# VikParuchuri/surya

Measured on AMD Instinct MI355X. Metric: text-lines/sec recognised (whole node), higher is better.
Workload: dtype bf16; 1 GPU; RecognitionPredictor device loop, 256 ragged 64x{128..512} crops/GPU, batch 256, max_tokens=48, REC-FULL synthetic weights (conditioned recipe, seed 0), tiles resident in HBM; parallelism=1 GPU, weights=conditioned

## Files before the change

### include/surya_amd.h

```cpp
#ifndef SURYA_AMD_H
#define SURYA_AMD_H
#include <stddef.h>
#include <stdint.h>

#ifdef __cplusplus
extern "C" {
#endif

#define SA_OK 0
#define SA_ERR_ARG (-1)
#define SA_ERR_SHAPE (-2)
#define SA_ERR_UNSUPPORTED (-3)
#define SA_ERR_STATE (-4)
#define SA_ERR_NOMEM (-5)

#define SA_DTYPE_F32 0
#define SA_DTYPE_BF16 1
#define SA_DTYPE_F16 2

const char* surya_amd_version(void);

typedef struct surya_rec_config {
    int32_t enc_depth, enc_hidden, enc_inter, enc_inter_pad, enc_heads;
    int32_t patch_dim, patch_dim_pad;
    int32_t merge;
    int32_t window_tokens;
    int32_t enc_out_hidden;
    uint32_t fullatt_mask;
    float enc_eps;
    int32_t vocab, dec_hidden, dec_inter, dec_layers, dec_heads, dec_kv_heads, dec_head_dim;
    float dec_eps;
    int32_t bbox_size, embed_multiplier;
    int32_t image_token_id, pad_token_id, eos_token_id;
    int32_t max_slots;
    int32_t max_kv_len;
    int32_t max_patches;
    int32_t max_prefill_tokens;
    int32_t dtype;
} surya_rec_config;

enum {
    SA_RW_PATCH = 0, SA_RW_MERGER_LN, SA_RW_FC1_W, SA_RW_FC1_B, SA_RW_FC2_W, SA_RW_FC2_B, SA_RW_IMG_H, SA_RW_IMG_W,
    SA_RW_DEC_NORM, SA_RW_TOK_EMBED, SA_RW_LM_W, SA_RW_LM_B, SA_RW_BBOX_W, SA_RW_BBOX_B, SA_RW_ENC_INVFREQ,
    SA_RW_DEC_INVFREQ, SA_RW_GLOBALS
};
enum { SA_RE_NORM1 = 0, SA_RE_QKV_W, SA_RE_QKV_B, SA_RE_PROJ_W, SA_RE_PROJ_B, SA_RE_NORM2, SA_RE_GU_W, SA_RE_GU_B,
       SA_RE_DOWN_W, SA_RE_DOWN_B, SA_RE_COUNT };
enum { SA_RD_LN1 = 0, SA_RD_QKV_W, SA_RD_QKV_B, SA_RD_O_W, SA_RD_LN2, SA_RD_GU_W, SA_RD_DOWN_W, SA_RD_COUNT };
#define SA_RW_ENC(l, k) (SA_RW_GLOBALS + (l) * SA_RE_COUNT + (k))
#define SA_RW_DEC(cfg_enc_depth, l, k) (SA_RW_GLOBALS + (cfg_enc_depth) * SA_RE_COUNT + (l) * SA_RD_COUNT + (k))
#define SA_RW_TOTAL(enc_depth, dec_layers) (SA_RW_GLOBALS + (enc_depth) * SA_RE_COUNT + (dec_layers) * SA_RD_COUNT)

typedef struct surya_rec surya_rec;

size_t surya_rec_workspace_bytes(const surya_rec_config* cfg);

int surya_rec_create(const surya_rec_config* cfg, const void* const* weights, int n_weights, surya_rec** out);
int surya_rec_destroy(surya_rec* h);

int surya_rec_plan_encoder(const surya_rec_config* cfg, const int32_t* grid_hw, int n_images, int32_t* src_row,
                           int32_t* pos_hw, int32_t* cu_window, int32_t* n_windows, int32_t* merged_src);

int surya_rec_prefill(surya_rec* h, const float* tiles, const int32_t* grid_hw, int n_images, const int32_t* input_ids,
                      const int32_t* seq_offsets, const int32_t* slot_ids, int n_seqs, void* stream);

int surya_rec_encode_ahead(surya_rec* h, const float* tiles, const int32_t* grid_hw, int n_images, void* stream);

int surya_rec_set_active(surya_rec* h, const int32_t* slots, int n_active, void* stream);

#define SA_MAX_STEPS 16
int surya_rec_decode(surya_rec* h, int n_steps, void* stream);

int surya_rec_read_outputs(surya_rec* h, int n_steps, int32_t* tokens, float* scores, int32_t* bboxes, void* stream);

int surya_rec_decode_async(surya_rec* h, int n_steps, int ring, void* stream);
int surya_rec_wait_outputs(surya_rec* h, int n_steps, int ring, int32_t* tokens, float* scores, int32_t* bboxes);

int surya_rec_preprocess(const uint8_t* pages, const void* lines, int n_lines, uint8_t* mask_arena, float* mid_arena, float* tiles,
                         int patch_size, int merge_size, float pad_value, const float* mean, const float* std, int any_poly,
                         int max_stage1_width, int pixel_stride, void* stream);

int surya_rec_encode_only(surya_rec* h, const float* tiles, const int32_t* grid_hw, int n_images, void* out, void* stream);
int surya_rec_copy_last_logits(surya_rec* h, float* dst, int max_rows, int* rows, void* stream);
int surya_rec_set_next_tokens(surya_rec* h, const int32_t* slots, const int32_t* tokens, int n, void* stream);

enum { SA_MX_QKV_W = 0, SA_MX_QKV_S, SA_MX_O_W, SA_MX_O_S, SA_MX_GU_W, SA_MX_GU_S, SA_MX_DOWN_W, SA_MX_DOWN_S, SA_MX_COUNT };
enum { SA_MX_LM_W = 0, SA_MX_LM_S, SA_MX_GLOBALS };
#define SA_MX_TOTAL(dec_layers) ((dec_layers) * SA_MX_COUNT + SA_MX_GLOBALS)
int surya_rec_set_mx_weights(surya_rec* h, const void* const* table, int n);

int surya_rec_set_kv_fp8(surya_rec* h, int on);

int surya_op_gemm(int dtype, int out_f32, int epi, const void* X, long ldx, const void* W, long ldw, void* C, long ldc,
                  const void* bias, const void* R, long ldr, int M, int N, int K, void* stream);
int surya_op_rmsnorm(int dtype, const void* x, long ldx, const void* w, void* y, long ldy, int rows, int C, float eps,
                     void* stream);
int surya_op_attn(int dtype, int head_dim, const void* q, const void* k, const void* v, void* out, const int32_t* seg_len,
                  const int64_t* q_off, const int64_t* k_off, const int64_t* v_off, const int64_t* o_off, int n_seg, int heads, int group,
                  int causal, float scale, long q_row, long q_head, long k_row, long k_head, long o_row, long o_head, void* stream);
int surya_op_decode_attn(int dtype, int head_dim, const float* qkv_part, int n_slabs, const void* qkv_bias, void* out, void* kcache,
                         void* vcache, const int32_t* active_slots, const int32_t* row_len, const float* rope_cs, int rows, int heads,
                         int kv_heads, int max_kv_len, float scale, void* stream);
int surya_op_kv8_quant_rows(int head_dim, const void* kcache, const void* vcache, const int32_t* tok_slot, const int32_t* tok_pos, int n_tokens,
                            void* k8, void* v8t, float* kscale, float* vscale, int kv_heads, int max_kv_len, void* stream);
int surya_op_decode_attn_kv8(int head_dim, const float* qkv_part, int n_slabs, const void* qkv_bias, void* out, void* k8, void* v8t,
                             float* kscale, float* vscale, const int32_t* active_slots, const int32_t* row_len, const float* rope_cs, int rows,
                             int heads, int kv_heads, int max_kv_len, float scale, void* stream);

int surya_op_gemm_splitk_bf16(const void* X, long ldx, const void* W, long ldw, float* part, int M, int N, int K, int* splitk, void* stream);
int surya_op_mx_quantize(const float* x, int rows, int K, uint8_t* q, uint8_t* scales, void* stream);
int surya_op_gemm_mx(int mode, const uint8_t* X, const uint8_t* SX, const uint8_t* W, const uint8_t* SW, int M, int N, int K,
                     float* C, int* splitk, uint8_t* q_out, uint8_t* sq_out, void* stream);

enum { SA_DET_INPUT = 0,
       SA_DET_CONV,
       SA_DET_DWCONV,
       SA_DET_GROUPED1X1,
       SA_DET_LITEMLA,
       SA_DET_UPCAT,
       SA_DET_CLASSIFY,
       SA_DET_UPSAMPLE_OUT,
       SA_DET_UPSUM_SRC,
       SA_DET_UPSUM_CLASSIFY };
enum { SA_ACT_NONE = 0, SA_ACT_HSWISH = 1, SA_ACT_RELU = 2 };

typedef struct surya_det_op {
    int32_t type;
    int32_t in0, in1, out, res;
    int32_t cin, cout, k, stride, act;
    int32_t hin, win, hout, wout;
    int32_t w_idx, b_idx;
    int32_t p0, p1;
} surya_det_op;

typedef struct surya_det_config {
    int32_t n_ops, max_batch, height, width, num_labels, dtype;
} surya_det_config;

typedef struct surya_det surya_det;

int surya_det_create(const surya_det_config* cfg, const surya_det_op* ops, const void* const* weights, int n_weights,
                     const size_t* buf_elems, int n_bufs, surya_det** out);
int surya_det_destroy(surya_det* h);
int surya_det_forward(surya_det* h, const float* pixel_values, int batch, float* heatmaps, float* lowres, void* stream);
int surya_det_op_count(surya_det* h);
int surya_det_forward_timed(surya_det* h, const float* pixel_values, int batch, float* heatmaps, float* lowres, void* stream, float* op_ms,
                            int n_op_ms);
int surya_det_forward_u8(surya_det* h, const uint8_t* pixels_nhwc, int pixel_stride, const float* mean, const float* std, int batch,
                         float* heatmaps, float* lowres, void* stream);

int surya_resample_lanczos_u8(const uint8_t* src, int src_w, int src_h, int src_pix, uint8_t* dst, int dst_w, int dst_h, int dst_pix,
                              const int32_t* bounds_x, const int32_t* taps_x, int ksize_x, const int32_t* bounds_y,
                              const int32_t* taps_y, int ksize_y, uint8_t* tmp, void* stream);

size_t surya_det_boxes_workspace_bytes(int batch, int height, int width, int max_boxes);
int surya_det_boxes(const float* heat, long page_stride, int batch, int height, int width, float text_threshold, float low_text,
                    int max_boxes, float* boxes, float* conf, int32_t* count, void* workspace, size_t workspace_bytes, void* stream);

typedef struct surya_layout_config {
    int32_t img_h, img_w, patch, embed_dim, n_stages;
    int32_t depths[8], heads[8], kv_heads[8];
    int32_t window;
    float enc_eps;
    int32_t encoder_length;
    int32_t dec_layers, dec_hidden, dec_inter, dec_heads, dec_kv_heads;
    int32_t vocab, label_count, bbox_size;
// ... 63 lines not shown
```

### surya_amd/csrc/attn_mfma.h

```cpp
#pragma once
#include "common.h"
#include "kernels.h"

namespace sa {

typedef short s16x4 __attribute__((ext_vector_type(4)));

template <int D>
__global__ __launch_bounds__(128) void attn_mfma_kernel(const bf16_t* __restrict__ q, const bf16_t* __restrict__ k,
                                                        const bf16_t* __restrict__ v, bf16_t* __restrict__ out, AttnSegs sg,
                                                        long q_row, long q_head, long k_row, long k_head, long o_row, long o_head,
                                                        int group, int causal, float scale) {
    static_assert(D % 16 == 0 && D <= 128, "head dim");
    constexpr int KC = 64;
    constexpr int PK = D + 8;
    constexpr int NKK = D / 16;
    constexpr int NDB = (D + 31) / 32;
    constexpr int CPR = D / 8;
    __shared__ __attribute__((aligned(16))) bf16_t ks[(KC + 1) * PK];
    __shared__ __attribute__((aligned(16))) bf16_t vs[(KC + 1) * PK];

    const int tile = blockIdx.x, head = blockIdx.y, kvh = head / group;
    const int seg = sg.tile_seg[tile], q0 = sg.tile_q0[tile], L = sg.seg_len[seg];
    const int tid = threadIdx.x, lane = tid & 63, wave = tid >> 6;
    const int ql = lane & 31, h = lane >> 5;
    const int qi = q0 + wave * 32 + ql;

    u32x4 qf[NKK];
    {
        const bf16_t* qp = q + sg.q_off[seg] + (long)min(qi, L - 1) * q_row + (long)head * q_head + h * 8;
#pragma unroll
        for (int kk = 0; kk < NKK; ++kk) qf[kk] = *reinterpret_cast<const u32x4*>(qp + kk * 16);
    }
    f32x16 oacc[NDB];
#pragma unroll
    for (int db = 0; db < NDB; ++db)
#pragma unroll
        for (int r = 0; r < 16; ++r) oacc[db][r] = 0.f;
    float mrun = -INFINITY, lrun = 0.f;
    const float sl2 = scale * 1.44269504088896340736f;

    const int kend = causal ? min(L, q0 + 64) : L;
    const bf16_t* kbase = k + sg.k_off[seg] + (long)kvh * k_head;
    const bf16_t* vbase = v + sg.v_off[seg] + (long)kvh * k_head;
    const int tr_off = ((lane & 15) >> 2) * PK + ((lane >> 4) & 1) * 16 + (lane & 3) * 4 + h * 4 * PK;

    constexpr int NST = KC * CPR / 128;
    static_assert(KC * CPR % 128 == 0, "staging split");
    u32x4 kreg[NST], vreg[NST];
    auto fetch = [&](int kc) {
        const int nk = min(KC, kend - kc);
#pragma unroll
        for (int it = 0; it < NST; ++it) {
            const int c = tid + it * 128, r = min(c / CPR, nk - 1), cc = c % CPR;
            kreg[it] = *reinterpret_cast<const u32x4*>(kbase + (long)(kc + r) * k_row + cc * 8);
            vreg[it] = *reinterpret_cast<const u32x4*>(vbase + (long)(kc + r) * k_row + cc * 8);
        }
    };
    if (kend > 0) fetch(0);
    for (int kc = 0; kc < kend; kc += KC) {
        const int nk = min(KC, kend - kc);
#pragma unroll
        for (int it = 0; it < NST; ++it) {
            const int c = tid + it * 128, r = c / CPR, cc = c % CPR;
            const bool in = r < nk;
            const u32x4 z = {0u, 0u, 0u, 0u};
            *reinterpret_cast<u32x4*>(ks + r * PK + cc * 8) = in ? kreg[it] : z;
            *reinterpret_cast<u32x4*>(vs + r * PK + cc * 8) = in ? vreg[it] : z;
        }
        __syncthreads();
        if (kc + KC < kend) fetch(kc + KC);

        f32x16 sacc[2];
#pragma unroll
        for (int kb = 0; kb < 2; ++kb) {
#pragma unroll
            for (int r = 0; r < 16; ++r) sacc[kb][r] = 0.f;
            const bf16_t* kp = ks + (kb * 32 + ql) * PK + h * 8;
#pragma unroll
            for (int kk = 0; kk < NKK; ++kk) {
                const u32x4 kf = *reinterpret_cast<const u32x4*>(kp + kk * 16);
                sacc[kb] = __builtin_amdgcn_mfma_f32_32x32x16_bf16(__builtin_bit_cast(bf16x8, kf), __builtin_bit_cast(bf16x8, qf[kk]),
                                                                   sacc[kb], 0, 0, 0);
            }
        }
        float bm = -INFINITY;
#pragma unroll
        for (int kb = 0; kb < 2; ++kb)
#pragma unroll
            for (int g = 0; g < 4; ++g)
#pragma unroll
                for (int r = 0; r < 4; ++r) {
                    const int j = kb * 32 + g * 8 + h * 4 + r;
                    const bool ok = (j < nk) && (!causal || (kc + j) <= qi);
                    const float sv = ok ? sacc[kb][4 * g + r] : -INFINITY;
                    sacc[kb][4 * g + r] = sv;
                    bm = fmaxf(bm, sv);
                }
        bm = fmaxf(bm, __shfl_xor(bm, 32, 64));
        const float mnew = fmaxf(mrun, bm);
        const float alpha = exp2f((mrun - mnew) * sl2);
        mrun = mnew;
        float psum = 0.f;
#pragma unroll
        for (int kb = 0; kb < 2; ++kb)
#pragma unroll
            for (int r = 0; r < 16; ++r) {
                const float pv = exp2f((sacc[kb][r] - mnew) * sl2);
                sacc[kb][r] = pv;
                psum += pv;
            }
        lrun = lrun * alpha + psum;
#pragma unroll
        for (int db = 0; db < NDB; ++db)
#pragma unroll
            for (int r = 0; r < 16; ++r) oacc[db][r] *= alpha;

#pragma unroll
        for (int t = 0; t < 4; ++t) {
            const int kb = t >> 1, o8 = (t & 1) * 8;
            u32x4 pf;
            pf[0] = pack2(sacc[kb][o8 + 0], sacc[kb][o8 + 1]);
            pf[1] = pack2(sacc[kb][o8 + 2], sacc[kb][o8 + 3]);
            pf[2] = pack2(sacc[kb][o8 + 4], sacc[kb][o8 + 5]);
            pf[3] = pack2(sacc[kb][o8 + 6], sacc[kb][o8 + 7]);
#pragma unroll
            for (int db = 0; db < NDB; ++db) {
                const bf16_t* vp = vs + t * 16 * PK + db * 32 + tr_off;
                const s16x4 lo = __builtin_amdgcn_ds_read_tr16_b64_v4i16((__attribute__((address_space(3))) s16x4*)(vp));
                const s16x4 hi = __builtin_amdgcn_ds_read_tr16_b64_v4i16((__attribute__((address_space(3))) s16x4*)(vp + 8 * PK));
                typedef short s16x8 __attribute__((ext_vector_type(8)));
                const s16x8 vf = __builtin_shufflevector(lo, hi, 0, 1, 2, 3, 4, 5, 6, 7);
                oacc[db] = __builtin_amdgcn_mfma_f32_32x32x16_bf16(__builtin_bit_cast(bf16x8, vf), __builtin_bit_cast(bf16x8, pf),
                                                                   oacc[db], 0, 0, 0);
            }
        }
        __syncthreads();
    }

    const float ltot = lrun + __shfl_xor(lrun, 32, 64);
    if (qi < L) {
        const float inv = 1.0f / ltot;
        bf16_t* op = out + sg.o_off[seg] + (long)qi * o_row + (long)head * o_head;
#pragma unroll
        for (int db = 0; db < NDB; ++db)
#pragma unroll
            for (int g = 0; g < 4; ++g) {
                const int d0 = db * 32 + g * 8 + h * 4;
                if (d0 < D) store4(op + d0, oacc[db][4 * g] * inv, oacc[db][4 * g + 1] * inv, oacc[db][4 * g + 2] * inv,
                                   oacc[db][4 * g + 3] * inv);
            }
    }
}

}
```

### surya_amd/csrc/common.h

```cpp
#pragma once
#include <hip/hip_runtime.h>
#include <cstdlib>
#include <stdint.h>
#include <stdio.h>

#include "../../include/surya_amd.h"

namespace sa {

typedef unsigned short bf16_t;
typedef __attribute__((ext_vector_type(4))) float f32x4;
typedef __attribute__((ext_vector_type(16))) float f32x16;
typedef __attribute__((ext_vector_type(8))) __bf16 bf16x8;
typedef unsigned int u32x4 __attribute__((ext_vector_type(4)));


#define SA_HIP(expr)                                                                                   \
    do {                                                                                               \
        hipError_t _e = (expr);                                                                        \
        if (_e != hipSuccess) {                                                                        \
            fprintf(stderr, "[surya_amd] %s:%d %s -> %s\n", __FILE__, __LINE__, #expr, hipGetErrorString(_e)); \
            return (int)_e;                                                                            \
        }                                                                                              \
    } while (0)
// ... 144 lines not shown
    const float m = oct_max(fmaxf(fmaxf(fabsf(v[0]), fabsf(v[1])), fmaxf(fabsf(v[2]), fabsf(v[3]))));
    const int e = mx_block_exp(m);
    e8 = e + 127;
    return mx_pack4(ldexpf(v[0], -e), ldexpf(v[1], -e), ldexpf(v[2], -e), ldexpf(v[3], -e));
}

__device__ __forceinline__ float wave_sum(float v) {
#pragma unroll
    for (int o = 32; o > 0; o >>= 1) v += __shfl_xor(v, o, 64);
    return v;
}
__device__ __forceinline__ float wave_max(float v) {
#pragma unroll
    for (int o = 32; o > 0; o >>= 1) v = fmaxf(v, __shfl_xor(v, o, 64));
    return v;
}

__device__ __forceinline__ float silu_f(float x) { return x / (1.0f + __expf(-x)); }
template <typename TI>
__device__ __forceinline__ float silu_epi(float x) {
    if constexpr (sizeof(TI) == 2) return x * __builtin_amdgcn_rcpf(1.0f + __expf(-x));
    else return silu_f(x);
}
__device__ __forceinline__ float gelu_erf_f(float x) { return 0.5f * x * (1.0f + erff(x * 0.70710678118654752440f)); }
template <typename TI>
__device__ __forceinline__ float gelu_epi(float x) {
    if constexpr (sizeof(TI) == 2) {
        const float z = fabsf(x) * 0.70710678118654752440f;
        const float t = __builtin_amdgcn_rcpf(fmaf(0.3275911f, z, 1.0f));
        const float poly = t * fmaf(t, fmaf(t, fmaf(t, fmaf(t, 1.061405429f, -1.453152027f), 1.421413741f), -0.284496736f), 0.254829592f);
        const float erfc_abs = poly * __expf(-z * z);
        return 0.5f * x * (x < 0.f ? erfc_abs : 2.0f - erfc_abs);
    } else {
        return gelu_erf_f(x);
    }
}
__device__ __forceinline__ float gelu_tanh_f(float x) { return 0.5f * x * (1.0f + tanhf(0.7978845608028654f * (x + 0.044715f * x * x * x))); }
__device__ __forceinline__ float sigmoid_f(float x) { return 1.0f / (1.0f + __expf(-x)); }
__device__ __forceinline__ float hardswish_f(float x) {
    float t;
    asm("v_fma_f32 %0, %1, %2, 0.5 clamp" : "=v"(t) : "v"(x), "s"(1.0f / 6.0f));
    return x * t;
}
typedef float f32x2_hs __attribute__((ext_vector_type(2)));
__device__ __forceinline__ f32x2_hs hardswish_pk(f32x2_hs x) {
    f32x2_hs t;
    const f32x2_hs c = {1.0f / 6.0f, 1.0f / 6.0f};
    asm("v_pk_fma_f32 %0, %1, %2, 0.5 op_sel_hi:[1,0,0] clamp" : "=v"(t) : "v"(x), "s"(c));
    return x * t;
}

struct Tuning {
    int graph = 0;
    int split_target = 256;
    int split_min_kt = 4;
    int split_max = 8;
    int bigtile = 3;
    int bigtile_any = 0;
    int big_m_split = -1;
    int big_m_gateup = -1;
    int gateup_ring = 2;
    int dring = 1;
    int dring_min_kt = 0;
    int conv_persist = 3;
    int dwconv_pipe = 2;
    int conv_lean = 1;
    int bigtile_ratio_pct = 0;
    int bigtile_min_k = 0;
    int glds = 2;
    int dattn = 4;
    int rnorm = 2;
    int ghead = 2;
    int fuse_embed = 1;
    int kvprefetch = 0;
    int lmhead = 1;
    int dattn_db = 0;
    int lay_ln = 1;
    int det_head_blk = 1;
    int det_fuse = 1023;
    int det_up4 = 1;
    int fmb_chunk = 64;
    int persist = 1;
    int ocrerr_cls_only = 1;
};
inline Tuning& tuning() { static Tuning t; return t; }
inline int& tuning_epoch() { static int e = 0; return e; }

inline void poison_arena(void* p, size_t bytes) {
    static const bool on = [] { const char* e = getenv("SURYA_AMD_POISON"); return e && e[0] == '1'; }();
    if (on) { (void)hipMemset(p, 0xFF, bytes); (void)hipDeviceSynchronize(); }
}

struct AttrOnce {
    size_t granted[64] = {};
    template <typename F> void ensure(F kern, size_t lds) {
        int dev = 0;
        (void)hipGetDevice(&dev);
        size_t& g = granted[dev & 63];
        if (lds > g || g == 0) {
            (void)hipFuncSetAttribute(reinterpret_cast<const void*>(kern), hipFuncAttributeMaxDynamicSharedMemorySize, (int)lds);
            g = lds > g ? lds : g;
            if (g == 0) g = 1;
        }
    }
};

static inline int cdiv(int a, int b) { return (a + b - 1) / b; }
static inline long cdivl(long a, long b) { return (a + b - 1) / b; }

}
```

### surya_amd/csrc/gemm.h

```cpp
#pragma once
#include <algorithm>
#include <cstdlib>
#include <type_traits>

#include "common.h"
#include "fastdiv.h"

namespace sa {

enum GemmEpi { EPI_BIAS = 0, EPI_RESIDUAL = 1, EPI_GELU = 2, EPI_SWIGLU = 3, EPI_HARDSWISH = 4, EPI_RELU = 5, EPI_ARGMAX = 6, EPI_ROPE = 7,
               EPI_GEGLU = 8  };

template <typename TI, typename TO>
struct GemmArgs {
    const TI* X; long ldx;
    const TI* W; long ldw;
    TO* C; long ldc;
    const TI* bias;
    const TO* R; long ldr;
    int M, N, K;
    int splitk = 1;
    float* part = nullptr;
    int swz_m = 0, swz_n = 0;
    int mgroup = 0;
    float4* amax = nullptr;
    mutable int bn_used = 0;
    const float2* rope = nullptr;
    int rope_cols = 0, rope_D = 0;
    const TI* conv_in = nullptr;
    const TI* conv_zero = nullptr;
    int cH = 0, cW = 0, cCin = 0, cHo = 0, cWo = 0, cKW = 0, cStride = 0, cPad = 0, cTaps = 0;
    int conv_lean = 1;
    FastDiv fd_hw, fd_wo;
    unsigned cv_m1 = 0, cv_m2 = 0;
    int cv_rowskip = 0;
#ifndef SA_P8_TIMING
#define SA_P8_TIMING 0
#endif
#if SA_P8_TIMING
    long long* dbg = nullptr;
#endif
};

template <typename TI> struct Mfma;
template <> struct Mfma<bf16_t> {
    __device__ static __forceinline__ void run(f32x16& acc, const u32x4& w, const u32x4& x) { acc = H16<bf16_t>::mfma(w, x, acc); }
};
template <> struct Mfma<fp16_t> {
    __device__ static __forceinline__ void run(f32x16& acc, const u32x4& w, const u32x4& x) { acc = H16<fp16_t>::mfma(w, x, acc); }
};
template <> struct Mfma<float> {
    __device__ static __forceinline__ void run(f32x16& acc, const u32x4& w, const u32x4& x) {
        acc = __builtin_amdgcn_mfma_f32_32x32x2f32(__uint_as_float(w[0]), __uint_as_float(x[0]), acc, 0, 0, 0);
        acc = __builtin_amdgcn_mfma_f32_32x32x2f32(__uint_as_float(w[1]), __uint_as_float(x[1]), acc, 0, 0, 0);
        acc = __builtin_amdgcn_mfma_f32_32x32x2f32(__uint_as_float(w[2]), __uint_as_float(x[2]), acc, 0, 0, 0);
        acc = __builtin_amdgcn_mfma_f32_32x32x2f32(__uint_as_float(w[3]), __uint_as_float(x[3]), acc, 0, 0, 0);
    }
};

template <typename TI, typename TO, int BM, int BN, int WM, int WN, int EPI, bool SPLIT = false, int GLDS = 0, bool CONV = false, int WAUX = 0>
__global__ __launch_bounds__(64 * WM * WN) void gemm_nt_kernel(GemmArgs<TI, TO> p) {
    static_assert(!CONV || (GLDS == 2 && !SPLIT), "the convolution gather exists for the 2-stage direct-to-LDS loop");
    constexpr int NT = 64 * WM * WN;
    constexpr int KE = Ty<TI>::KE;
    constexpr int WTM = BM / WM, WTN = BN / WN;
    constexpr int FM = WTM / 32, FN = WTN / 32;
    constexpr int XCH = (BM * 8 + NT - 1) / NT, WCH = (BN * 8 + NT - 1) / NT;
    constexpr int XMOD = XCH * NT > BM * 8 ? BM * 8 : XCH * NT, WMOD = WCH * NT > BN * 8 ? BN * 8 : WCH * NT;
    static_assert(FM >= 1 && FN >= 1 && WTM % 32 == 0 && WTN % 32 == 0, "tile");
    static_assert((XCH == 1 || (BM * 8) % NT == 0) && (WCH == 1 || (BN * 8) % NT == 0), "staging split");
    extern __shared__ __attribute__((aligned(16))) unsigned char smem[];
    constexpr int XBYTES = BM * 128, WBYTES = BN * 128, BUF = XBYTES + WBYTES;

    const int tid = threadIdx.x, lane = tid & 63, wave = tid >> 6;
    const int wm = wave / WN, wn = wave % WN;
    const int tiles_n = (p.N + BN - 1) / BN;
    int tile_m = (int)blockIdx.x / tiles_n, tile_n = (int)blockIdx.x % tiles_n, ks = 0;
    if constexpr (SPLIT) {
        const int tiles_m = (p.M + BM - 1) / BM;
        const int x = (int)blockIdx.x & 7, j = (int)blockIdx.x >> 3;
        const int pair = (j / tiles_m) * 8 + x;
        if (pair >= tiles_n * p.splitk) return;
        tile_m = j % tiles_m;
        tile_n = pair / p.splitk;
        ks = pair % p.splitk;
    }
    if (!SPLIT && p.mgroup) {
        const int tiles_m = (p.M + BM - 1) / BM;
        const int x = (int)blockIdx.x & 7, j = (int)blockIdx.x >> 3;
        const int pair = (j / tiles_m) * 8 + x;
        if (pair >= tiles_n) return;
        tile_m = j % tiles_m;
        tile_n = pair;
    }
    if (!SPLIT && p.swz_n > 0) {
        const int x = (int)blockIdx.x & 7, j = (int)blockIdx.x >> 3;
        constexpr int GRP = ((BM + BN) * 128 * (GLDS > 2 && GLDS != 8 ? GLDS : 2) > 80 * 1024) ? 32 : 64;
        const int idx = ((j / GRP) * 8 + x) * GRP + (j % GRP);
        const int tiles_m = (p.M + BM - 1) / BM;
        if (idx >= tiles_m * tiles_n) return;
        const int per_row = p.swz_m * tiles_n;
        const int sr = idx / per_row, rem = idx - sr * per_row;
        const int h = min(p.swz_m, tiles_m - sr * p.swz_m);
        const int sc = rem / (h * p.swz_n), rem2 = rem - sc * h * p.swz_n;
        const int w = min(p.swz_n, tiles_n - sc * p.swz_n);
        tile_m = sr * p.swz_m + rem2 / w;
        tile_n = sc * p.swz_n + rem2 % w;
    }
    const int m0 = tile_m * BM, n0 = tile_n * BN;
#if SA_P8_TIMING
#define SA_STAMP1(IDX) { if (p.dbg && tid == 0) p.dbg[(long)blockIdx.x * 4 + (IDX)] = (long long)__builtin_readcyclecounter(); }
#else
#define SA_STAMP1(IDX) {}
#endif
    SA_STAMP1(0);
    const int nk_all = p.K / KE;
    const int kt_begin = SPLIT ? (int)((long)ks * nk_all / p.splitk) : 0;
    const int kt_end = SPLIT ? (int)((long)(ks + 1) * nk_all / p.splitk) : nk_all;
// ... 855 lines not shown
        int nt_m = 0, nt_n = 0;
        const bool have_next = next_tile(nt_m, nt_n);
        set_req(tile_m, tile_n);
        set_read();
        if constexpr (CONV && EPI == EPI_RESIDUAL) { set_conv(tile_m, 0, 0); set_conv(tile_m, 0, 1); set_conv(tile_m, 1, 0); set_conv(tile_m, 1, 1); }
        if (wv >= 4) __builtin_amdgcn_s_barrier();
        __builtin_amdgcn_sched_barrier(0);
        SP_STAMP(0);
        {
            SP_PHASE({ SP_RX(xa, 0); SP_RW(1); }, SP_REQX(1, 6, 1), -1, xa, 0, 0, true);
            SP_PHASE(SP_RX(xb, 2), SP_REQW(1, 7, 1), -1, xb, 0, 1, true);
            SP_PHASE(SP_RW(3),     SP_REQX(0, 0, 2), -1, xb, 1, 1, true);
            SP_PHASE(SP_RX(xb, 4), SP_REQW(0, 1, 2), -1, xa, 1, 0, true);
            SP_STAMP(1);
            SP_PHASE(SP_RW(5),     SP_REQX(1, 2, 2),  8, xb, 0, 0, false);
            SP_STAMP(2);
            SP_PHASE(SP_RX(xa, 6), SP_REQW(1, 3, 2),  8, xa, 0, 1, false);
            SP_PHASE(SP_RW(7),     SP_REQX(0, 4, 3),  8, xa, 1, 1, false);
            SP_PHASE(SP_RX(xa, 0), SP_REQW(0, 5, 3),  8, xb, 1, 0, false);
        }
        SP_STAMP(3);
        for (int pi = 1; pi < pairs - 1; ++pi) {
            const int t = 2 * pi;
            SP_PHASE(SP_RW(1),     SP_REQX(1, 6, t + 1), 8, xa, 0, 0, false);
            SP_PHASE(SP_RX(xb, 2), SP_REQW(1, 7, t + 1), 8, xb, 0, 1, false);
            SP_PHASE(SP_RW(3),     SP_REQX(0, 0, t + 2), 8, xb, 1, 1, false);
            SP_PHASE(SP_RX(xb, 4), SP_REQW(0, 1, t + 2), 8, xa, 1, 0, false);
            SP_PHASE(SP_RW(5),     SP_REQX(1, 2, t + 2), 8, xb, 0, 0, false);
            SP_PHASE(SP_RX(xa, 6), SP_REQW(1, 3, t + 2), 8, xa, 0, 1, false);
            SP_PHASE(SP_RW(7),     SP_REQX(0, 4, t + 3), 8, xa, 1, 1, false);
            SP_PHASE(SP_RX(xa, 0), SP_REQW(0, 5, t + 3), 8, xb, 1, 0, false);
        }
        SP_STAMP(4);
        unsigned bpack_raw = 0, bias_mask = 0;
        {
            const int t = nk - 2;
            if constexpr (CONV) { if (have_next) set_conv(nt_m, 0, 0); }
            SP_PHASE(SP_RW(1),     SP_REQX(1, 6, t + 1), 8, xa, 0, 0, false);
            if constexpr (CONV) { if (have_next) set_conv(nt_m, 0, 1); }
            SP_PHASE(SP_RX(xb, 2), SP_REQW(1, 7, t + 1), 8, xb, 0, 1, false);
            SP_STAMP(9);
            if (have_next) set_req(nt_m, nt_n);
            if constexpr (CONV) { if (have_next) set_conv(nt_m, 1, 0); }
            SP_STAMP(10);
            SP_PHASE(SP_RW(3),     { if (have_next) { SP_REQX(0, 0, 0); SP_VM(8); } else { SP_VM(6); } }, -1, xb, 1, 1, false);
            SP_STAMP(11);
            if constexpr (CONV) { if (have_next) set_conv(nt_m, 1, 1); }
            SP_PHASE(SP_RX(xb, 4), { if (have_next) { SP_REQW(0, 1, 0); SP_VM(8); } else { SP_VM(4); } }, -1, xa, 1, 0, false);
            SP_PHASE(SP_RW(5),     { if (have_next) { SP_REQX(1, 2, 0); SP_VM(8); } else { SP_VM(2); } }, -1, xb, 0, 0, false);
            SP_PHASE(SP_RX(xa, 6), { if (have_next) { SP_REQW(1, 3, 0); SP_VM(8); } else { SP_VM(0); } }, -1, xa, 0, 1, false);
            SP_PHASE(SP_RW(7),     { if (have_next) { SP_REQX(0, 4, 1); SP_VM(8); } },                    -1, xa, 1, 1, false);
            const TI* bias_p = p.bias ? p.bias : p.W;
            bias_mask = p.bias ? 0xffffffffu : 0u;
            bpack_raw = *reinterpret_cast<const unsigned*>(bias_p + min(n0 + wn * 128 + 2 * fresh_lane(), p.N - 2));
            SP_PHASE({},           { if (have_next) { SP_REQW(0, 5, 1); SP_VM(8); } },                    -1, xb, 1, 0, false);
            if (wv < 4) __builtin_amdgcn_s_barrier();
        }

        SP_STAMP(5);
        constexpr bool GLU = (EPI == EPI_SWIGLU || EPI == EPI_GEGLU);
        const int n_out = GLU ? p.N / 2 : p.N, n0_out = GLU ? n0 / 2 : n0;
        const int lane_e = fresh_lane();
        const int srow = lane_e & 31, lhi = lane_e >> 5;
        constexpr int NBLK = GLU ? 2 : 4;
        const int rrow = lane_e >> 3, rc = lane_e & 7;
        [[maybe_unused]] u32x4 res[NBLK][4];
        [[maybe_unused]] const unsigned char* r_tile = reinterpret_cast<const unsigned char*>(p.R + (long)m0 * p.ldr + n0_out);
        unsigned char* c_tile = reinterpret_cast<unsigned char*>(p.C + (long)m0 * p.ldc + n0_out);
        const int rows_left = p.M - m0, cols_left = n_out - n0_out;
        if constexpr (EPI == EPI_RESIDUAL) {
#pragma unroll
            for (int blk = 0; blk < NBLK; ++blk)
#pragma unroll
                for (int it = 0; it < 4; ++it) {
                    const int rl = min(wm * 64 + (blk >> 1) * 32 + it * 8 + rrow, rows_left - 1), cl = min(wn * 128 + (blk & 1) * 64 + rc * 8, cols_left - 8);
                    res[blk][it] = *reinterpret_cast<const u32x4*>(r_tile + (unsigned)(rl * (int)(p.ldr * sizeof(TO)) + cl * (int)sizeof(TO)));
                }
        }
        __builtin_amdgcn_sched_barrier(0);
        typedef unsigned int u32x2 __attribute__((ext_vector_type(2)));
        using Pk = typename std::conditional<GLU, unsigned, u32x2>::type;
        const unsigned bpack = bpack_raw & bias_mask;
        Pk pk[4][2][4];
#pragma unroll
        for (int jp = 0; jp < 2; ++jp)
#pragma unroll
            for (int i = 0; i < 2; ++i) {
                [[maybe_unused]] float4 rope_v[2][4];
                if constexpr (EPI == EPI_ROPE) {
                    const int m = min(m0 + wm * 64 + i * 32 + srow, p.M - 1), half = p.rope_D >> 1;
#pragma unroll
                    for (int j2 = 0; j2 < 2; ++j2)
#pragma unroll
                        for (int g = 0; g < 4; ++g) {
                            const int n = min(min(n0 + wn * 128 + (jp * 2 + j2) * 32 + g * 8 + lhi * 4, p.N - 4), p.rope_cols - 4);
                            rope_v[j2][g] = *reinterpret_cast<const float4*>(p.rope + (long)m * half + ((n % p.rope_D) >> 1));
                        }
                }
#pragma unroll
                for (int j2 = 0; j2 < 2; ++j2)
#pragma unroll
                    for (int g = 0; g < 4; ++g) {
                        const int j = jp * 2 + j2;
                        const int wcol = j * 32 + g * 8 + lhi * 4;
                        const unsigned lo = (unsigned)__builtin_amdgcn_ds_bpermute((wcol >> 1) << 2, (int)bpack), hi = (unsigned)__builtin_amdgcn_ds_bpermute(((wcol >> 1) + 1) << 2, (int)bpack);
                        float v[4] = {acc[j][i][4 * g], acc[j][i][4 * g + 1], acc[j][i][4 * g + 2], acc[j][i][4 * g + 3]};
                        v[0] += H16<TI>::lo(lo); v[1] += H16<TI>::hi(lo);
                        v[2] += H16<TI>::lo(hi); v[3] += H16<TI>::hi(hi);
                        if constexpr (EPI == EPI_GELU) {
#pragma unroll
                            for (int r = 0; r < 4; ++r) v[r] = gelu_epi<TI>(v[r]);
                        } else if constexpr (EPI == EPI_HARDSWISH) {
#pragma unroll
                            for (int r = 0; r < 4; ++r) v[r] = hardswish_f(v[r]);
                        } else if constexpr (EPI == EPI_RELU) {
#pragma unroll
                            for (int r = 0; r < 4; ++r) v[r] = fmaxf(v[r], 0.f);
                        }
                        if constexpr (EPI == EPI_ROPE) {
                            const int n = min(n0 + wn * 128 + wcol, p.N - 4);
                            if (n < p.rope_cols) {
                                const float4 cs = rope_v[j2][g];
                                const float x0 = Ty<TO>::rnd(v[0]), x1 = Ty<TO>::rnd(v[1]), x2 = Ty<TO>::rnd(v[2]), x3 = Ty<TO>::rnd(v[3]);
                                v[0] = __fmaf_rn(x0, cs.x, -__fmul_rn(x1, cs.y)); v[1] = __fmaf_rn(x1, cs.x, __fmul_rn(x0, cs.y));
                                v[2] = __fmaf_rn(x2, cs.z, -__fmul_rn(x3, cs.w)); v[3] = __fmaf_rn(x3, cs.z, __fmul_rn(x2, cs.w));
                            }
                        }
                        if constexpr (GLU) {
                            if constexpr (EPI == EPI_GEGLU) {
                                const float g0 = Ty<TO>::rnd(gelu_tanh_f(Ty<TO>::rnd(v[0]))), g1 = Ty<TO>::rnd(gelu_tanh_f(Ty<TO>::rnd(v[2])));
                                pk[j][i][g] = H16<TO>::pk(g0 * Ty<TO>::rnd(v[1]), g1 * Ty<TO>::rnd(v[3]));
                            } else {
                                pk[j][i][g] = H16<TO>::pk(silu_epi<TI>(v[0]) * v[1], silu_epi<TI>(v[2]) * v[3]);
                            }
                        } else {
                            pk[j][i][g] = Pk{H16<TO>::pk(v[0], v[1]), H16<TO>::pk(v[2], v[3])};
                        }
                    }
            }
        __builtin_amdgcn_sched_barrier(0);
        SP_STAMP(6);
        SP_VM(0);
        SP_STAMP(7);
        __builtin_amdgcn_sched_barrier(0);
#pragma unroll
        for (int blk = 0; blk < NBLK; ++blk) {
            const int i = GLU ? blk : blk >> 1, jh = GLU ? 0 : blk & 1;
            const int cl = wn * (GLU ? 64 : 128) + jh * 64 + rc * 8;
            if constexpr (GLU) {
#pragma unroll
                for (int j2 = 0; j2 < 4; ++j2)
#pragma unroll
                    for (int gp = 0; gp < 2; ++gp) {
                        const auto sw = __builtin_amdgcn_permlane32_swap(pk[j2][i][2 * gp], pk[j2][i][2 * gp + 1], false, false);
                        const int boff = (j2 * 16 + gp * 8 + lhi * 4) * (int)sizeof(TO);
                        typedef unsigned int u32x2s __attribute__((ext_vector_type(2)));
                        *reinterpret_cast<u32x2s*>(stage + srow * 128 + ((((boff >> 4) ^ (srow & 7)) << 4) | (boff & 15))) = u32x2s{sw[0], sw[1]};
                    }
            } else {
#pragma unroll
                for (int j2 = 0; j2 < 2; ++j2)
#pragma unroll
                    for (int g = 0; g < 4; ++g) {
                        const int boff = (j2 * 32 + g * 8 + lhi * 4) * (int)sizeof(TO);
                        *reinterpret_cast<Pk*>(stage + srow * 128 + ((((boff >> 4) ^ (srow & 7)) << 4) | (boff & 15))) = pk[jh * 2 + j2][i][g];
                    }
            }
            u32x4 raw[4];
#pragma unroll
            for (int it = 0; it < 4; ++it) {
                const int r = it * 8 + rrow;
                raw[it] = *reinterpret_cast<const u32x4*>(stage + r * 128 + ((rc ^ (r & 7)) << 4));
            }
#pragma unroll
            for (int it = 0; it < 4; ++it) {
                const int rl = wm * 64 + i * 32 + it * 8 + rrow;
                if (rl >= rows_left || cl >= cols_left) continue;
                TO* dst = reinterpret_cast<TO*>(c_tile + (unsigned)(rl * (int)(p.ldc * sizeof(TO)) + cl * (int)sizeof(TO)));
                if constexpr (EPI == EPI_RESIDUAL) {
                    float a[8], r8[8];
                    unpack16(make_uint4(raw[it][0], raw[it][1], raw[it][2], raw[it][3]), a, (TO*)nullptr);
                    unpack16(make_uint4(res[blk][it][0], res[blk][it][1], res[blk][it][2], res[blk][it][3]), r8, (TO*)nullptr);
#pragma unroll
                    for (int e = 0; e < 8; e += 4) store4(dst + e, a[e] + r8[e], a[e + 1] + r8[e + 1], a[e + 2] + r8[e + 2], a[e + 3] + r8[e + 3]);
                    __builtin_amdgcn_sched_barrier(0);
                } else {
                    *reinterpret_cast<u32x4*>(dst) = raw[it];
                }
            }
        }
        SP_STAMP(8);
#if SA_P8_TIMING
        ++dbg_tile;
#endif
        if (!have_next) return;
        tile_m = nt_m; tile_n = nt_n;
    }
#undef SP_STAMP
#undef SP_PHASE
#undef SP_VM
#undef SP_MMA
#undef SP_RW
#undef SP_RX
#undef SP_REQX
#undef SP_REQW
#undef SP_REQ
}
#undef SA_COMPUTE
#undef SA_COMPUTE_FULL
#undef SA_COMPUTE_LEAN
#undef SA_FRAGS
#undef SA_MFMAS

struct GemmProfiler {
    static constexpr int NCFG = 4, POOL = 8192;
    bool enabled = false;
    hipEvent_t ev[2 * POOL];
    bool have_events = false;
    int n = 0;
    int cfg_of[POOL];
    double flops_of[POOL], bytes_of[POOL], slab_of[POOL];
    void start() {
        if (!have_events) {
            for (int i = 0; i < 2 * POOL; ++i) (void)hipEventCreate(&ev[i]);
            have_events = true;
        }
        n = 0; enabled = true;
    }
};
inline GemmProfiler& gemm_profiler() { static GemmProfiler p; return p; }
inline int gemm_cfg_id(int BM, int BN) { return (BM >= 128 && BN >= 128) ? 0 : (BM == 256 ? 1 : 2); }

template <typename TI, typename TO, int BM, int BN, int WM, int WN, int EPI, bool SPLIT = false, int GLDS = 0, bool CONV = false, int WAUX = 0>
static inline int launch_gemm_cfg(const GemmArgs<TI, TO>& a, hipStream_t s) {
    int tiles = SPLIT ? cdiv(cdiv(a.N, BN) * a.splitk, 8) * 8 * cdiv(a.M, BM) : cdiv(a.M, BM) * cdiv(a.N, BN);
    a.bn_used = BN;
    GemmArgs<TI, TO> aa = a;
    if (!SPLIT && BM >= 128 && BN >= 128) {
        const int tm = cdiv(a.M, BM), tn = cdiv(a.N, BN);
        constexpr int GRP = ((BM + BN) * 128 * (GLDS > 2 && GLDS != 8 ? GLDS : 2) > 80 * 1024) ? 32 : 64;
        if (tm * tn >= 8 * GRP) {
            aa.swz_n = cdiv(tn, cdiv(tn, 8));
            aa.swz_m = std::max(1, GRP / aa.swz_n);
            tiles = cdiv(tm * tn, 8 * GRP) * 8 * GRP;
        }
    }
    if (!SPLIT && aa.mgroup) tiles = cdiv(cdiv(a.N, BN), 8) * 8 * cdiv(a.M, BM);
    constexpr size_t out_w = ((EPI == EPI_SWIGLU || EPI == EPI_GEGLU) && !SPLIT) ? BN / 2 : BN;
    constexpr size_t out_bytes = (size_t)BM * out_w * (SPLIT ? sizeof(float) : sizeof(TO));
    constexpr size_t stage_bytes = (size_t)(BM + BN) * 128 * (GLDS > 2 && GLDS != 8 ? GLDS : 2);
    constexpr bool argmax_direct = (EPI == EPI_ARGMAX) && ((size_t)BM * BN * 4 > 160 * 1024);
    constexpr size_t lds = (argmax_direct || stage_bytes > out_bytes) ? stage_bytes : out_bytes;
    auto kern = gemm_nt_kernel<TI, TO, BM, BN, WM, WN, EPI, SPLIT, GLDS, CONV, WAUX>;
    static AttrOnce attr;
    attr.ensure(kern, lds);
    GemmProfiler& pf = gemm_profiler();
    const bool prof = pf.enabled && pf.n < GemmProfiler::POOL;
    if (prof) (void)hipEventRecord(pf.ev[2 * pf.n], s);
    hipLaunchKernelGGL(kern, dim3(tiles), dim3(64 * WM * WN), lds, s, aa);
    if (prof) {
        (void)hipEventRecord(pf.ev[2 * pf.n + 1], s);
        pf.cfg_of[pf.n] = CONV ? 3 : gemm_cfg_id(BM, BN);
        pf.flops_of[pf.n] = CONV ? 2.0 * a.M * a.N * a.cTaps * a.cCin : 2.0 * a.M * a.N * a.K;
        const double outn = (EPI == EPI_SWIGLU || EPI == EPI_GEGLU) ? a.N / 2 : (EPI == EPI_ARGMAX ? 4.0 * cdiv(a.N, BN) : a.N);
        const double xelems = CONV ? (double)a.M / std::max(1, a.cHo * a.cWo) * a.cH * a.cW * a.cCin : (double)a.M * a.K;
        pf.bytes_of[pf.n] = (xelems + (double)a.N * a.K) * sizeof(TI) + (double)a.M * outn * (SPLIT ? sizeof(TI) : sizeof(TO)) +
                            (EPI == EPI_RESIDUAL ? (double)a.M * a.N * sizeof(TO) : 0.0);
        pf.slab_of[pf.n] = SPLIT ? (double)a.splitk * a.M * a.N * 4.0 : 0.0;
        ++pf.n;
    }
    return (int)hipGetLastError();
}

template <typename TI, typename TO, int EPI, int CONV = 0>
static inline int launch_gemm_persist(const GemmArgs<TI, TO>& a, hipStream_t s) {
    constexpr int BM = 256, BN = 256, GRP = 32;
    const int tm = cdiv(a.M, BM), tn = cdiv(a.N, BN);
    GemmArgs<TI, TO> aa = a;
    a.bn_used = BN;
    aa.swz_n = cdiv(tn, cdiv(tn, 8));
    aa.swz_m = std::max(1, GRP / aa.swz_n);
    const int padded = cdiv(tm * tn, 8 * GRP) * 8 * GRP;
    static int n_cu_of[64] = {};
    int dev = 0;
    (void)hipGetDevice(&dev);
    int& n_cu = n_cu_of[dev & 63];
    if (!n_cu) {
        if (hipDeviceGetAttribute(&n_cu, hipDeviceAttributeMultiprocessorCount, dev) != hipSuccess || n_cu <= 0) n_cu = 256;
        n_cu = (n_cu / 8) * 8;
    }
    const int grid = std::min(padded, n_cu);
    constexpr size_t lds = (size_t)2 * (BM + BN) * 128 + 8 * 4096;
    auto kern = gemm_nt_p8p_kernel<TI, TO, EPI, CONV>;
    static AttrOnce attr;
    attr.ensure(kern, lds);
    GemmProfiler& pf = gemm_profiler();
    const bool prof = pf.enabled && pf.n < GemmProfiler::POOL;
    if (prof) (void)hipEventRecord(pf.ev[2 * pf.n], s);
    hipLaunchKernelGGL(kern, dim3(grid), dim3(512), lds, s, aa);
    if (prof) {
        (void)hipEventRecord(pf.ev[2 * pf.n + 1], s);
        pf.cfg_of[pf.n] = CONV ? 3 : gemm_cfg_id(BM, BN);
        pf.flops_of[pf.n] = CONV ? 2.0 * a.M * a.N * a.cTaps * a.cCin : 2.0 * a.M * a.N * a.K;
        const double outn = (EPI == EPI_SWIGLU || EPI == EPI_GEGLU) ? a.N / 2 : a.N;
        const double xelems = CONV ? (double)a.M / std::max(1, a.cHo * a.cWo) * a.cH * a.cW * a.cCin : (double)a.M * a.K;
        pf.bytes_of[pf.n] = (xelems + (double)a.N * a.K) * sizeof(TI) + (double)a.M * outn * sizeof(TO) +
                            (EPI == EPI_RESIDUAL ? (double)a.M * a.N * sizeof(TO) : 0.0);
        pf.slab_of[pf.n] = 0.0;
        ++pf.n;
    }
    return (int)hipGetLastError();
}

}
#include "gemm_ring.h"
namespace sa {

template <typename TI, typename TO, int EPI>
static inline int launch_gemm(const GemmArgs<TI, TO>& a, hipStream_t s) {
    if (a.M <= 0 || a.N <= 0) return SA_OK;
    {
        const int n_out = (EPI == EPI_SWIGLU || EPI == EPI_GEGLU) ? a.N / 2 : a.N;
        if (a.K % Ty<TI>::KE != 0 || a.N % 4 != 0 || n_out % (16 / (int)sizeof(TO)) != 0 || a.ldc % (16 / (int)sizeof(TO)) != 0)
            return SA_ERR_SHAPE;
    }
    if (a.M <= 256) {
        if constexpr (EPI == EPI_ARGMAX) {
            if (a.N >= 64 * 512 && tuning().lmhead && (a.K / Ty<TI>::KE) % 2 == 0 && a.N % 4 == 0) {
                if constexpr (sizeof(TI) == 2)
                    if (tuning().lmhead == 2) return launch_gemm_cfg<TI, TO, 256, 320, 4, 2, EPI, false, 2, false, 2>(a, s);
                return launch_gemm_cfg<TI, TO, 256, 320, 4, 2, EPI, false, 2>(a, s);
            }
            if (a.N >= 64 * 512) return launch_gemm_cfg<TI, TO, 128, 128, 2, 2, EPI, false, 2>(a, s);
            return launch_gemm_cfg<TI, TO, 64, 64, 2, 2, EPI, false, 2>(a, s);
        }
        if (a.M > 128) {
            if (a.N >= 64 * 512) return launch_gemm_cfg<TI, TO, 128, 128, 2, 2, EPI, false, 2>(a, s);
            if constexpr (EPI == EPI_SWIGLU && sizeof(TI) == 2 && sizeof(TO) == 2) {
                const int rc = launch_gateup_ring(a, s);
                if (rc >= 0) return rc;
            }
            if constexpr (EPI == EPI_SWIGLU && sizeof(TI) == 2) {
                if (tuning().gateup_ring == 3) return launch_gemm_cfg<TI, TO, 64, 64, 2, 2, EPI, false, 3>(a, s);
                if (tuning().gateup_ring == 4) return launch_gemm_cfg<TI, TO, 64, 64, 2, 2, EPI, false, 4>(a, s);
            }
            return launch_gemm_cfg<TI, TO, 64, 64, 2, 2, EPI, false, 2>(a, s);
        }
        if (a.M > 64) {
            if (a.N >= 64 * 128) return launch_gemm_cfg<TI, TO, 128, 64, 4, 1, EPI>(a, s);
            return launch_gemm_cfg<TI, TO, 128, 32, 4, 1, EPI>(a, s);
        }
        if (a.N >= 64 * 128) return launch_gemm_cfg<TI, TO, 64, 64, 2, 2, EPI>(a, s);
        return launch_gemm_cfg<TI, TO, 64, 32, 2, 1, EPI>(a, s);
    }
    if constexpr (EPI == EPI_ARGMAX) {
        if (a.N >= 64 * 512 && tuning().lmhead && (a.K / Ty<TI>::KE) % 2 == 0 && a.N % 4 == 0) {
            GemmArgs<TI, TO> g = a;
            g.mgroup = 1;
            int rc;
            if constexpr (sizeof(TI) == 2) {
                if (tuning().lmhead == 2) { rc = launch_gemm_cfg<TI, TO, 256, 320, 4, 2, EPI, false, 2, false, 2>(g, s); a.bn_used = g.bn_used; return rc; }
            }
            rc = launch_gemm_cfg<TI, TO, 256, 320, 4, 2, EPI, false, 2>(g, s);
            a.bn_used = g.bn_used;
            return rc;
        }
    }
    if constexpr (EPI == EPI_SWIGLU && sizeof(TI) == 2 && sizeof(TO) == 2) {
        const int mode = tuning().big_m_gateup;
        const int rb = cdiv(a.M, 256), t256 = rb * cdiv(a.N, 256);
        const int pick = mode >= 0 ? mode : ((rb >= 4 && t256 >= 160 && t256 < 256) ? 2 : 0);
        if (pick && (a.K / Ty<TI>::KE) % 2 == 0 && a.K / Ty<TI>::KE >= 4 && a.N % 8 == 0) {
            if (pick == 1) return launch_gemm_persist<TI, TO, EPI>(a, s);
            return launch_gemm_cfg<TI, TO, 256, 256, 4, 2, EPI, false, 8>(a, s);
        }
    }
    if (a.N <= 64 && a.M >= 128 * 256) return launch_gemm_cfg<TI, TO, 128, 64, 4, 1, EPI>(a, s);
    const long big = (long)cdiv(a.M, 128) * cdiv(a.N, 128);
    const int glds = tuning().glds;
    if constexpr (sizeof(TO) == 2) {
        const int bigtile = tuning().bigtile;
        const long t256 = (long)cdiv(a.M, 256) * cdiv(a.N, 256);
        const double ratio256 = tuning().bigtile_ratio_pct > 0 ? tuning().bigtile_ratio_pct / 100.0
                                                                : ((bigtile == 3 && sizeof(TI) == 2) ? 1.4 : 1.17);
        const double cost256 = (double)cdivl(t256, 256) * 256 * 4 / ratio256, cost128 = (double)cdivl(big, 512) * 512;
        if (bigtile && a.K >= tuning().bigtile_min_k && ((t256 >= 256 && cost256 <= cost128) || tuning().bigtile_any)) {
            if constexpr (EPI != EPI_ARGMAX) {
                const int nk = a.K / Ty<TI>::KE;
                if constexpr (sizeof(TI) == 2)
                    if (tuning().persist && nk >= 4 && nk % 2 == 0 && a.N % 8 == 0) return launch_gemm_persist<TI, TO, EPI>(a, s);
            }
            if constexpr (sizeof(TI) == 2 && EPI != EPI_ARGMAX) {
                if (bigtile == 2) return launch_gemm_cfg<TI, TO, 256, 256, 2, 2, EPI, false, 2>(a, s);
                if (bigtile == 3 && (a.K / Ty<TI>::KE) % 2 == 0) return launch_gemm_cfg<TI, TO, 256, 256, 4, 2, EPI, false, 8>(a, s);
            }
            return launch_gemm_cfg<TI, TO, 256, 256, 4, 2, EPI, false, 2>(a, s);
        }
    }
    if (big >= 256) {
        if (glds == 2) return launch_gemm_cfg<TI, TO, 128, 128, 2, 2, EPI, false, 2>(a, s);
// ... 36 lines not shown
```

### surya_amd/csrc/kernels.h

```cpp
#pragma once
#include "common.h"

#ifndef SA_DBG_VARIANT
#define SA_DBG_VARIANT 0
#endif

namespace sa {

template <typename T>
__global__ void convert_tiles_kernel(const float* __restrict__ in, T* __restrict__ out, const int* __restrict__ src_row,
                                     int P, int kin, int kout) {
    const int row = blockIdx.x;
    const float* src = in + (long)src_row[row] * kin;
    T* dst = out + (long)row * kout;
    for (int c = threadIdx.x * 4; c < kout; c += blockDim.x * 4) {
        float v[4];
#pragma unroll
        for (int r = 0; r < 4; ++r) v[r] = (c + r < kin) ? src[c + r] : 0.f;
        store4(dst + c, v[0], v[1], v[2], v[3]);
    }
}

template <typename T>
__global__ __launch_bounds__(256) void rmsnorm_kernel(const T* __restrict__ x, long ldx, const T* __restrict__ w,
// ... 71 lines not shown
            load4(qp + i, t4);
#pragma unroll
            for (int r = 0; r < 4; ++r) qr[i + r] = t4[r] * scale;
        }
    }
#pragma unroll
    for (int i = 0; i < DS; ++i) acc[i] = 0.f;
    float mrun = -INFINITY, lrun = 0.f;
    const int kend = causal ? min(L, q0 + 64) : L;
    const T* kbase = k + sg.k_off[seg] + (long)kvh * k_head;
    const T* vbase = v + sg.v_off[seg] + (long)kvh * k_head;
    for (int kc = 0; kc < kend; kc += KC) {
        const int nk = min(KC, kend - kc);
        for (int c = tid; c < nk * CPR; c += 256) {
            const int r = c / CPR, cc = c % CPR;
            *reinterpret_cast<uint4*>(ks + r * D + cc * V) = *reinterpret_cast<const uint4*>(kbase + (long)(kc + r) * k_row + cc * V);
            *reinterpret_cast<uint4*>(vs + r * D + cc * V) = *reinterpret_cast<const uint4*>(vbase + (long)(kc + r) * k_row + cc * V);
        }
        __syncthreads();
        for (int jb = 0; jb < nk; jb += 16) {
            float s[16];
            float bm = -INFINITY;
#pragma unroll
            for (int jj = 0; jj < 16; ++jj) {
                const int j = jb + jj;
                float d = 0.f;
                if (j < nk) {
                    const T* kr = ks + j * D + sl * DS;
#pragma unroll
                    for (int i = 0; i < DS; i += 4) {
                        float t4[4];
                        load4(kr + i, t4);
                        d += qr[i] * t4[0] + qr[i + 1] * t4[1] + qr[i + 2] * t4[2] + qr[i + 3] * t4[3];
                    }
                }
                d = quad_sum(d);
                const bool ok = (j < nk) && (!causal || (kc + j) <= qi);
                s[jj] = ok ? d : -INFINITY;
                bm = fmaxf(bm, s[jj]);
            }
            if (bm == -INFINITY) continue;
            const float mnew = fmaxf(mrun, bm);
            const float alpha = __expf(mrun - mnew);
            lrun *= alpha;
#pragma unroll
            for (int i = 0; i < DS; ++i) acc[i] *= alpha;
            mrun = mnew;
#pragma unroll
            for (int jj = 0; jj < 16; ++jj) {
                const int j = jb + jj;
                if (j < nk) {
                    const float pj = __expf(s[jj] - mnew);
                    lrun += pj;
                    const T* vr = vs + j * D + sl * DS;
#pragma unroll
                    for (int i = 0; i < DS; i += 4) {
                        float t4[4];
                        load4(vr + i, t4);
                        acc[i] += pj * t4[0]; acc[i + 1] += pj * t4[1]; acc[i + 2] += pj * t4[2]; acc[i + 3] += pj * t4[3];
                    }
                }
            }
        }
        __syncthreads();
    }
    if (valid) {
        const float inv = 1.0f / lrun;
        T* op = out + sg.o_off[seg] + (long)qi * o_row + (long)head * o_head + sl * DS;
#pragma unroll
        for (int i = 0; i < DS; i += 4) store4(op + i, acc[i] * inv, acc[i + 1] * inv, acc[i + 2] * inv, acc[i + 3] * inv);
    }
}

template <typename T>
__global__ void scatter_rows_kernel(const T* __restrict__ src, const int* __restrict__ dst_row, T* __restrict__ dst, int H) {
    const int r = blockIdx.x;
    const T* s = src + (long)r * H;
    T* d = dst + (long)dst_row[r] * H;
    for (int c = threadIdx.x * Ty<T>::V16; c < H; c += blockDim.x * Ty<T>::V16)
        *reinterpret_cast<uint4*>(d + c) = *reinterpret_cast<const uint4*>(s + c);
}

template <typename T>
__global__ void scatter_image_kernel(const T* __restrict__ merged, const T* __restrict__ hemb, const T* __restrict__ wemb,
                                     const int* __restrict__ dst_row, const int* __restrict__ hidx, const int* __restrict__ widx,
                                     T* __restrict__ embeds, int H) {
    const int r = blockIdx.x;
    const T* src = merged + (long)r * H;
    const T* he = hemb + (long)hidx[r] * H;
    const T* we = wemb + (long)widx[r] * H;
    T* dst = embeds + (long)dst_row[r] * H;
    for (int c = threadIdx.x * 4; c < H; c += blockDim.x * 4) {
        float a[4], b[4], d[4];
        load4(src + c, a); load4(he + c, b); load4(we + c, d);
        store4(dst + c, a[0] + Ty<T>::rnd(b[0] + d[0]), a[1] + Ty<T>::rnd(b[1] + d[1]), a[2] + Ty<T>::rnd(b[2] + d[2]),
               a[3] + Ty<T>::rnd(b[3] + d[3]));
    }
}

template <typename T>
__global__ void embed_tokens_kernel(const T* __restrict__ table, const int* __restrict__ ids, T* __restrict__ x, int H) {
    const int t = blockIdx.x;
    const int id = ids[t];
    if (id < 0) return;
    const uint4* src = reinterpret_cast<const uint4*>(table + (long)id * H);
    uint4* dst = reinterpret_cast<uint4*>(x + (long)t * H);
    for (int c = threadIdx.x; c < H / Ty<T>::V16; c += blockDim.x) dst[c] = src[c];
}

template <typename T>
__global__ void rope_table_kernel(const float* __restrict__ inv_freq, float2* __restrict__ table, int Tmax, int half) {
    const int idx = blockIdx.x * blockDim.x + threadIdx.x;
    if (idx >= Tmax * half) return;
    const int pos = idx / half, i = idx % half;
    float sn, cs;
    sincosf((float)pos * inv_freq[i], &sn, &cs);
    table[idx] = make_float2(Ty<T>::rnd(cs), Ty<T>::rnd(sn));
}

template <typename T>
__global__ void rope_kv_append_kernel(T* __restrict__ qkv, const int* __restrict__ tok_slot, const int* __restrict__ tok_pos,
                                      const float2* __restrict__ rope_cs, T* __restrict__ kc, T* __restrict__ vc,
                                      int nq, int nkv, int D, int Tmax) {
    const int t = blockIdx.x;
    const int slot = tok_slot[t], pos = tok_pos[t];
    const int half = D / 2;
    T* row = qkv + (long)t * (nq + 2 * nkv) * D;
    for (int it = threadIdx.x; it < (nq + nkv) * half; it += blockDim.x) {
        const int i = it % half, hh = it / half;
        const float2 csn = rope_cs[(long)pos * half + i];
        const float cs = csn.x, sn = csn.y;
        T* v = row + (long)hh * D;
        const float x1 = Ty<T>::ld(v + i), x2 = Ty<T>::ld(v + i + half);
        const float y1 = x1 * cs - x2 * sn, y2 = x2 * cs + x1 * sn;
        if (hh < nq) {
            Ty<T>::st(v + i, y1); Ty<T>::st(v + i + half, y2);
        } else {
            T* dst = kc + (((long)slot * nkv + (hh - nq)) * Tmax + pos) * D;
            Ty<T>::st(dst + i, y1); Ty<T>::st(dst + i + half, y2);
        }
    }
    const T* vsrc = row + (long)(nq + nkv) * D;
    for (int it = threadIdx.x; it < nkv * D; it += blockDim.x) {
        const int hh = it / D, i = it % D;
        vc[(((long)slot * nkv + hh) * Tmax + pos) * D + i] = vsrc[it];
    }
}

struct KvPrefetch {
    const unsigned char* base = nullptr;
    const int* slots = nullptr;
    const int* lens = nullptr;
    long slot_stride = 0, head_stride = 0;
    int heads = 0, row_bytes = 0, max_rows = 0;
};

template <typename T, int SL = 8>
__global__ __launch_bounds__(1024) void splitk_residual_norm_kernel(const float* __restrict__ part, int S, int M, T* __restrict__ x,
                                                                    const T* __restrict__ bias, const T* __restrict__ w,
                                                                    T* __restrict__ y, int H, float eps,
                                                                    uint8_t* __restrict__ y8 = nullptr, uint8_t* __restrict__ sy = nullptr,
                                                                    int srows = 0, KvPrefetch pf = KvPrefetch()) {
    if ((int)blockIdx.x >= M) {
        if (pf.base) {
            const int r = (int)blockIdx.x - M, t16 = (int)threadIdx.x * 16, step = (int)blockDim.x * 16;
            const int bytes = min(pf.lens[r] + 1, pf.max_rows) * pf.row_bytes;
            const unsigned char* p0 = pf.base + (long)pf.slots[r] * pf.slot_stride + t16;
            const int per_head = bytes > t16 ? (bytes - t16 + step - 1) / step : 0;
            const int total = per_head * pf.heads;
            u32x4 acc = {0u, 0u, 0u, 0u};
            int k = 0;
            const unsigned char* p = p0;
#pragma unroll 8
            for (int i = 0; i < total; ++i) {
                acc ^= *reinterpret_cast<const u32x4*>(p + (long)k * step);
                if (++k == per_head) { k = 0; p += pf.head_stride; }
            }
            asm volatile("" ::"v"(acc));
        }
        return;
    }
    const int row = blockIdx.x, tid = threadIdx.x;
    __shared__ float red[16];
    T* xr = x + (long)row * H;
    const int c = tid * 4;
    const bool on_row = c < H;
    const int cc = on_row ? c : 0;
    float v[4], g[4] = {0.f, 0.f, 0.f, 0.f};
    load4(xr + cc, v);
    if (w) load4(w + cc, g);
    if (bias) {
        float b[4];
        load4(bias + cc, b);
        v[0] += b[0]; v[1] += b[1]; v[2] += b[2]; v[3] += b[3];
    }
    f32x4 p4[SL];
#pragma unroll
    for (int s = 0; s < SL; ++s)
        p4[s] = *reinterpret_cast<const f32x4*>(part + ((long)min(s, S - 1) * M + row) * H + cc);
#pragma unroll
    for (int s = 0; s < SL; ++s) {
        const float on = (s < S) ? 1.f : 0.f;
        v[0] += on * p4[s][0]; v[1] += on * p4[s][1]; v[2] += on * p4[s][2]; v[3] += on * p4[s][3];
    }
    float ss = 0.f;
#pragma unroll
    for (int i = 0; i < 4; ++i) { v[i] = Ty<T>::rnd(v[i]); ss += on_row ? v[i] * v[i] : 0.f; }
    if (on_row) store4(xr + c, v[0], v[1], v[2], v[3]);
    if (!w) return;
    ss = wave_sum(ss);
    if ((tid & 63) == 0) red[tid >> 6] = ss;
    __syncthreads();
    float tot = 0.f;
    for (int i = 0; i < (int)(blockDim.x >> 6); ++i) tot += red[i];
    const float rstd = rsqrtf(tot / (float)H + eps);
    const float o[4] = {g[0] * Ty<T>::rnd(v[0] * rstd), g[1] * Ty<T>::rnd(v[1] * rstd), g[2] * Ty<T>::rnd(v[2] * rstd),
                        g[3] * Ty<T>::rnd(v[3] * rstd)};
// ... 284 lines not shown
```

### surya_amd/csrc/rec_model.hip

```cpp
#include <algorithm>
#include <cstdlib>
#include <cstring>
#include <map>
#include <memory>
#include <set>
#include <vector>

#include "../../include/surya_amd.h"
#include "gemm.h"
#include "gemm_mx.h"
#include "kernels.h"
#include "decode_attn.h"
#include "decode_attn_kv8.h"
#include "attn_mfma.h"
#include "rec_prep.h"

namespace sa {

struct Stager {
    char* host = nullptr;
    char* dev = nullptr;
    size_t cap = 0, off = 0;
    hipEvent_t ev = nullptr;
    bool pending = false;
// ... 33 lines not shown
    }
};

struct EncPlan {
    int P = 0;
    std::vector<int> src_row, pos_hw, merged_src, hidx, widx;
    std::vector<int> win_cu, img_cu;
};

static int plan_encoder(const surya_rec_config& c, const int32_t* grid_hw, int n, EncPlan& pl) {
    const int mg = c.merge, unit = mg * mg, vw = c.window_tokens;
    pl = EncPlan();
    pl.win_cu.push_back(0);
    pl.img_cu.push_back(0);
    int tok_base = 0;
    for (int im = 0; im < n; ++im) {
        const int h = grid_hw[2 * im], w = grid_hw[2 * im + 1];
        if (h <= 0 || w <= 0 || h % mg || w % mg) return SA_ERR_SHAPE;
        const int lh = h / mg, lw = w / mg;
        const int pad_h = vw - lh % vw, pad_w = vw - lw % vw;
        const int nh = (lh + pad_h) / vw, nw = (lw + pad_w) / vw;
        for (int wy = 0; wy < nh; ++wy)
            for (int wx = 0; wx < nw; ++wx) {
                int cnt = 0;
                for (int dy = 0; dy < vw; ++dy)
                    for (int dx = 0; dx < vw; ++dx) {
                        const int y = wy * vw + dy, x = wx * vw + dx;
                        if (y >= lh || x >= lw) continue;
                        const int tok = y * lw + x;
                        pl.merged_src.push_back(tok_base + tok);
                        pl.hidx.push_back((int)(((float)y / (float)std::max(1, lh - 1)) * (float)c.embed_multiplier));
                        pl.widx.push_back((int)(((float)x / (float)std::max(1, lw - 1)) * (float)c.embed_multiplier));
                        for (int u = 0; u < unit; ++u) {
                            pl.src_row.push_back((tok_base + tok) * unit + u);
                            pl.pos_hw.push_back(y * mg + u / mg);
                            pl.pos_hw.push_back(x * mg + u % mg);
                        }
                        ++cnt;
                    }
                if (cnt) pl.win_cu.push_back(pl.win_cu.back() + cnt * unit);
            }
        tok_base += lh * lw;
        pl.img_cu.push_back(pl.img_cu.back() + h * w);
    }
    pl.P = pl.img_cu.back();
    return SA_OK;
}

struct SegLists {
    std::vector<int> tile_seg, tile_q0, seg_len;
    std::vector<long> q_off, k_off, v_off, o_off;
    void add_tiles(int seg, int L) {
        for (int q0 = 0; q0 < L; q0 += 64) { tile_seg.push_back(seg); tile_q0.push_back(q0); }
    }
};

static AttnSegs stage_segs(Stager& st, const SegLists& s) {
    AttnSegs a;
    a.tile_seg = st.put(s.tile_seg); a.tile_q0 = st.put(s.tile_q0); a.seg_len = st.put(s.seg_len);
    a.q_off = st.put(s.q_off); a.k_off = st.put(s.k_off); a.v_off = st.put(s.v_off); a.o_off = st.put(s.o_off);
    return a;
}

__global__ void set_slot_state_kernel(const int* slots, const int* lens, int* kv_len, int n) {
    const int i = blockIdx.x * blockDim.x + threadIdx.x;
    if (i < n) kv_len[slots[i]] = lens[i];
}
__global__ void set_next_tokens_kernel(const int* slots, const int* toks, int* next_token, int n) {
    const int i = blockIdx.x * blockDim.x + threadIdx.x;
    if (i < n) next_token[slots[i]] = toks[i];
}

struct RecBase {
    virtual ~RecBase() {}
    virtual int prefill(const float*, const int32_t*, int, const int32_t*, const int32_t*, const int32_t*, int, hipStream_t) = 0;
    virtual int set_active(const int32_t*, int, hipStream_t) = 0;
    virtual int encode_ahead(const float*, const int32_t*, int, hipStream_t) = 0;
    virtual int decode(int, hipStream_t) = 0;
    virtual int read_outputs(int, int32_t*, float*, int32_t*, hipStream_t) = 0;
    virtual int decode_async(int, int, hipStream_t) = 0;
    virtual int wait_outputs(int, int, int32_t*, float*, int32_t*) = 0;
    virtual int encode_only(const float*, const int32_t*, int, void*, hipStream_t) = 0;
    virtual int copy_last_logits(float*, int, int*, hipStream_t) = 0;
    virtual int set_next_tokens(const int32_t*, const int32_t*, int, hipStream_t) = 0;
    virtual int set_mx_weights(const void* const*, int) = 0;
    virtual int set_kv_fp8(int) = 0;
};

static size_t align_up(size_t v) { return (v + 255) & ~(size_t)255; }

template <typename T>
struct RecModel : RecBase {
    surya_rec_config c;
    std::vector<const void*> w;
    char* arena = nullptr;
    size_t arena_bytes = 0;
    Stager st, st_small, st_enc;
    hipStream_t estream = nullptr;
    hipEvent_t ev_ahead_in = nullptr, ev_ahead_done = nullptr, ev_ahead_free = nullptr;
    T* emb_ahead = nullptr;
    long ahead_tokens = 0, ahead_consumed = 0;
    bool ahead_free_recorded = false;
    T *tiles_t, *ex, *eh, *eqkv, *emlp, *emh, *emerged;
    T *dx, *dh, *dqkv, *dattn, *dmlp, *dlast;
    float* logits;
    float2* erope;
    float4* amax;
    float2* rope_cs;
    float* part;
    T *kcache, *vcache;
    int *kv_len, *next_token, *active_dev, *row_len;
    int* out_token; float* out_score; int* out_bbox;
    char* out_host = nullptr;
    size_t out_bytes = 0;
    int n_active = 0;
    int last_rows = 0;
    bool last_heads_mx = false;
    hipStream_t gstream = nullptr;
    hipEvent_t gev_in = nullptr, gev_out = nullptr;
    hipEvent_t ev_ring[2] = {nullptr, nullptr};
    std::map<long, hipGraphExec_t> graphs;
    std::set<long> seen_keys;
    bool use_graph = true;
    int graph_epoch = 0;
    std::vector<int> h_len, h_active;
    int ctx_bound = 0;
    std::vector<const uint8_t*> mxw;
    char* mx_arena = nullptr;
    char* kv8_arena = nullptr;
    uint8_t *k8c = nullptr, *v8tc = nullptr;
    float *ksc8 = nullptr, *vsc8 = nullptr;
    bool kv8 = false;
    int tmax8() const { return (c.max_kv_len + 255) & ~255; }
    uint8_t *dh8 = nullptr, *sdh = nullptr, *dattn8 = nullptr, *sattn = nullptr, *dmlp8 = nullptr, *smlp = nullptr, *dlast8 = nullptr,
            *slast = nullptr;
    bool mx() const { return !mxw.empty(); }
    const uint8_t* MXW(int l, int k) const { return mxw[(size_t)l * SA_MX_COUNT + k]; }
    const uint8_t* MXG(int k) const { return mxw[(size_t)c.dec_layers * SA_MX_COUNT + k]; }

    const T* W(int idx) const { return reinterpret_cast<const T*>(w[idx]); }
    const T* WE(int l, int k) const { return W(SA_RW_ENC(l, k)); }
    const T* WD(int l, int k) const { return W(SA_RW_DEC(c.enc_depth, l, k)); }

    static size_t layout(const surya_rec_config& c, RecModel* m) {
        size_t off = 0;
        auto take = [&](size_t bytes) { size_t o = off; off = align_up(off + bytes); return o; };
        const size_t Pm = c.max_patches, Tm = std::max(c.max_prefill_tokens, c.max_slots), S = c.max_slots;
        const int unit = c.merge * c.merge;
        const size_t qkv_d = (size_t)(c.dec_heads + 2 * c.dec_kv_heads) * c.dec_head_dim;
        size_t o_tiles = take(Pm * c.patch_dim_pad * sizeof(T));
        size_t o_ex = take(Pm * c.enc_hidden * sizeof(T));
        size_t o_eh = take(Pm * c.enc_hidden * sizeof(T));
        size_t o_eqkv = take(Pm * 3 * c.enc_hidden * sizeof(T));
        size_t o_emlp = take(Pm * c.enc_inter_pad * sizeof(T));
        size_t o_emh = take(Pm * c.enc_hidden * sizeof(T));
        size_t o_erope = take(Pm * (size_t)(c.enc_hidden / c.enc_heads / 2) * sizeof(float2));
        size_t o_emerged = take(Pm / unit * c.enc_out_hidden * sizeof(T));
        size_t o_dx = take(Tm * c.dec_hidden * sizeof(T));
        size_t o_dh = take(Tm * c.dec_hidden * sizeof(T));
        size_t o_dqkv = take(Tm * qkv_d * sizeof(T));
        size_t o_dattn = take(Tm * c.dec_heads * c.dec_head_dim * sizeof(T));
        size_t o_dmlp = take(Tm * c.dec_inter * sizeof(T));
        size_t o_dlast = take(S * c.dec_hidden * sizeof(T));
        size_t o_ahead = take(Tm * c.dec_hidden * sizeof(T));
        size_t o_logits = take(S * (size_t)c.vocab * sizeof(float));
        size_t o_amax = take(S * (size_t)cdiv(c.vocab, 32) * sizeof(float4));
// ... 17 lines not shown
            m->kcache = (T*)(b + o_k); m->vcache = (T*)(b + o_v);
            m->kv_len = (int*)(b + o_kvlen); m->next_token = (int*)(b + o_next); m->active_dev = (int*)(b + o_active); m->row_len = (int*)(b + o_rowlen);
            m->out_token = (int*)(b + o_out);
            m->out_score = (float*)(m->out_token + (size_t)SA_MAX_STEPS * S);
            m->out_bbox = (int*)(m->out_score + (size_t)SA_MAX_STEPS * S);
            m->out_bytes = (size_t)SA_MAX_STEPS * S * 8 * sizeof(int);
        }
        return off;
    }

    int init(const surya_rec_config& cfg, const void* const* weights, int n) {
        c = cfg;
        w.assign(weights, weights + n);
        arena_bytes = layout(c, nullptr);
        SA_HIP(hipMalloc((void**)&arena, arena_bytes));
        poison_arena(arena, arena_bytes);
        layout(c, this);
        {
            const int half = c.dec_head_dim / 2, n = c.max_kv_len * half;
            hipLaunchKernelGGL(rope_table_kernel<T>, dim3(cdiv(n, 256)), dim3(256), 0, 0,
                               reinterpret_cast<const float*>(w[SA_RW_DEC_INVFREQ]), rope_cs, c.max_kv_len, half);
            SA_HIP(hipGetLastError());
        }
        SA_HIP(hipMemset(kv_len, 0, c.max_slots * sizeof(int)));
        SA_HIP(hipMemset(next_token, 0, c.max_slots * sizeof(int)));
        SA_HIP(hipMemset(out_token, 0, out_bytes));
        SA_HIP(hipHostMalloc((void**)&out_host, out_bytes, hipHostMallocDefault));
        const size_t Pm = c.max_patches, Tm = std::max(c.max_prefill_tokens, c.max_slots);
        int rc = st.init((Pm * 8 + Tm * 8 + (size_t)c.max_slots * 64) * sizeof(int) + (1 << 20));
        if (rc) return rc;
        rc = st_small.init((size_t)c.max_slots * 4 * sizeof(int) + 4096);
        if (rc) return rc;
        rc = st_enc.init((Pm * 8 + (size_t)c.max_slots * 64) * sizeof(int) + (1 << 20));
        if (rc) return rc;
        {
            int least = 0, greatest = 0;
            SA_HIP(hipDeviceGetStreamPriorityRange(&least, &greatest));
            SA_HIP(hipStreamCreateWithPriority(&estream, hipStreamNonBlocking, least));
            SA_HIP(hipEventCreateWithFlags(&ev_ahead_in, hipEventDisableTiming));
            SA_HIP(hipEventCreateWithFlags(&ev_ahead_done, hipEventDisableTiming));
            SA_HIP(hipEventCreateWithFlags(&ev_ahead_free, hipEventDisableTiming));
        }
        SA_HIP(hipStreamCreateWithFlags(&gstream, hipStreamNonBlocking));
        SA_HIP(hipEventCreateWithFlags(&gev_in, hipEventDisableTiming));
        SA_HIP(hipEventCreateWithFlags(&gev_out, hipEventDisableTiming));
        for (auto& e : ev_ring) SA_HIP(hipEventCreateWithFlags(&e, hipEventDisableTiming));
        use_graph = true;
        SA_HIP(hipDeviceSynchronize());
        return SA_OK;
    }
    ~RecModel() override {
        if (mx_arena) (void)hipFree(mx_arena);
        if (kv8_arena) (void)hipFree(kv8_arena);
        for (auto& kv : graphs) (void)hipGraphExecDestroy(kv.second);
        if (gstream) (void)hipStreamDestroy(gstream);
        if (gev_in) (void)hipEventDestroy(gev_in);
        if (gev_out) (void)hipEventDestroy(gev_out);
        for (auto e : ev_ring) if (e) (void)hipEventDestroy(e);
        st.destroy(); st_small.destroy(); st_enc.destroy();
        if (estream) (void)hipStreamDestroy(estream);
        for (hipEvent_t e : {ev_ahead_in, ev_ahead_done, ev_ahead_free}) if (e) (void)hipEventDestroy(e);
        if (arena) (void)hipFree(arena);
        if (out_host) (void)hipHostFree(out_host);
    }

    template <int EPI>
    int gemm(const T* X, long ldx, const T* Wt, long ldw, T* C, long ldc, const T* bias, const T* R, long ldr, int M, int N,
             int K, hipStream_t s) {
        GemmArgs<T, T> a{X, ldx, Wt, ldw, C, ldc, bias, R, ldr, M, N, K};
        return launch_gemm<T, T, EPI>(a, s);
    }
    int rmsnorm(const T* x, long ldx, const T* wt, T* y, long ldy, const int* src_row, int rows, int C, float eps, hipStream_t s) {
        if (rows <= 0) return SA_OK;
        hipLaunchKernelGGL(rmsnorm_kernel<T>, dim3(cdiv(rows, 4)), dim3(256), 0, s, x, ldx, wt, y, ldy, src_row, rows, C, eps);
        return (int)hipGetLastError();
    }
    int attention(int D, const T* q, const T* k, const T* v, T* o, const AttnSegs& sg, int n_tiles, int heads, long q_row,
                  long q_head, long k_row, long k_head, long o_row, long o_head, int group, int causal, float scale,
                  hipStream_t s) {
        if (n_tiles <= 0) return SA_OK;
        dim3 grid(n_tiles, heads), block(256);
        if constexpr (std::is_same<T, bf16_t>::value) {
            {
#define SA_ATTN_M(DD)                                                                                                    \
    hipLaunchKernelGGL((attn_mfma_kernel<DD>), grid, dim3(128), 0, s, q, k, v, o, sg, q_row, q_head, k_row, k_head, o_row, \
                       o_head, group, causal, scale)
                switch (D) {
                    case 32: SA_ATTN_M(32); break;
                    case 64: SA_ATTN_M(64); break;
                    case 80: SA_ATTN_M(80); break;
                    case 128: SA_ATTN_M(128); break;
                    default: return SA_ERR_UNSUPPORTED;
                }
#undef SA_ATTN_M
                return (int)hipGetLastError();
            }
        }
#define SA_ATTN(DD)                                                                                                    \
    hipLaunchKernelGGL((attn_valu_kernel<T, DD>), grid, block, 0, s, q, k, v, o, sg, q_row, q_head, k_row, k_head, o_row, \
                       o_head, group, causal, scale)
        switch (D) {
            case 32: SA_ATTN(32); break;
            case 64: SA_ATTN(64); break;
            case 80: SA_ATTN(80); break;
            case 128: SA_ATTN(128); break;
            default: return SA_ERR_UNSUPPORTED;
        }
#undef SA_ATTN
        return (int)hipGetLastError();
    }

    int encode(const float* tiles, const int32_t* grid_hw, int n, const std::vector<int>& dst_rows, T* dst, hipStream_t s) {
        return encode(tiles, grid_hw, n, dst_rows, dst, s, st);
    }
    int encode(const float* tiles, const int32_t* grid_hw, int n, const std::vector<int>& dst_rows, T* dst, hipStream_t s,
               Stager& st) {
        const int unit = c.merge * c.merge, He = c.enc_hidden, D = He / c.enc_heads;
        int i0 = 0;
        long patch_base = 0, tok_base = 0;
        while (i0 < n) {
            int i1 = i0;
            long P = 0;
            while (i1 < n) {
                const long p = (long)grid_hw[2 * i1] * grid_hw[2 * i1 + 1];
                if (p > c.max_patches) return SA_ERR_SHAPE;
                if (P + p > c.max_patches) break;
                P += p; ++i1;
            }
            EncPlan pl;
            int rc = plan_encoder(c, grid_hw + 2 * i0, i1 - i0, pl);
            if (rc) return rc;
            SegLists win, full;
            for (size_t sgi = 0; sgi + 1 < pl.win_cu.size(); ++sgi) {
                const int a = pl.win_cu[sgi], L = pl.win_cu[sgi + 1] - a;
                win.seg_len.push_back(L);
                win.q_off.push_back((long)a * 3 * He); win.k_off.push_back((long)a * 3 * He + He);
                win.v_off.push_back((long)a * 3 * He + 2 * He); win.o_off.push_back((long)a * He);
                win.add_tiles((int)sgi, L);
            }
            for (size_t sgi = 0; sgi + 1 < pl.img_cu.size(); ++sgi) {
                const int a = pl.img_cu[sgi], L = pl.img_cu[sgi + 1] - a;
                full.seg_len.push_back(L);
                full.q_off.push_back((long)a * 3 * He); full.k_off.push_back((long)a * 3 * He + He);
                full.v_off.push_back((long)a * 3 * He + 2 * He); full.o_off.push_back((long)a * He);
                full.add_tiles((int)sgi, L);
            }
            std::vector<int> dst_row(pl.merged_src.size());
            for (size_t g = 0; g < dst_row.size(); ++g) dst_row[g] = dst_rows[tok_base + pl.merged_src[g]];
            st.begin();
            const int* d_src_row = st.put(pl.src_row);
            const int* d_pos = st.put(pl.pos_hw);
            const int* d_dst = st.put(dst_row);
            const int* d_hidx = st.put(pl.hidx);
            const int* d_widx = st.put(pl.widx);
            AttnSegs d_win = stage_segs(st, win), d_full = stage_segs(st, full);
            if (!d_full.o_off) return SA_ERR_NOMEM;
            rc = st.flush(s);
            if (rc) return rc;

            const int Pi = (int)P;
            hipLaunchKernelGGL(convert_tiles_kernel<T>, dim3(Pi), dim3(64), 0, s, tiles + patch_base * c.patch_dim, tiles_t,
                               d_src_row, Pi, c.patch_dim, c.patch_dim_pad);
            if ((rc = gemm<EPI_BIAS>(tiles_t, c.patch_dim_pad, W(SA_RW_PATCH), c.patch_dim_pad, ex, He, nullptr, nullptr, 0, Pi,
                                     He, c.patch_dim_pad, s))) return rc;
            const float scale = 1.0f / sqrtf((float)D);
            hipLaunchKernelGGL(rope_vision_table_kernel, dim3((unsigned)cdivl((long)Pi * (D / 2), 256)), dim3(256), 0, s, d_pos,
                               reinterpret_cast<const float*>(w[SA_RW_ENC_INVFREQ]), erope, Pi, D);
            for (int l = 0; l < c.enc_depth; ++l) {
                if ((rc = rmsnorm(ex, He, WE(l, SA_RE_NORM1), eh, He, nullptr, Pi, He, c.enc_eps, s))) return rc;
                {
                    GemmArgs<T, T> a{eh, He, WE(l, SA_RE_QKV_W), He, eqkv, 3 * He, WE(l, SA_RE_QKV_B), nullptr, 0, Pi, 3 * He, He};
                    a.rope = erope; a.rope_cols = 2 * He; a.rope_D = D;
                    if ((rc = launch_gemm<T, T, EPI_ROPE>(a, s))) return rc;
                }
                const bool fullatt = (c.fullatt_mask >> l) & 1u;
                const AttnSegs& sg = fullatt ? d_full : d_win;
                const int nt = (int)(fullatt ? full.tile_seg.size() : win.tile_seg.size());
                if ((rc = attention(D, eqkv, eqkv, eqkv, eh, sg, nt, c.enc_heads, 3 * He, D, 3 * He, D, He, D, 1, 0, scale, s)))
                    return rc;
                if ((rc = gemm<EPI_RESIDUAL>(eh, He, WE(l, SA_RE_PROJ_W), He, ex, He, WE(l, SA_RE_PROJ_B), ex, He, Pi, He, He, s)))
                    return rc;
                if ((rc = rmsnorm(ex, He, WE(l, SA_RE_NORM2), eh, He, nullptr, Pi, He, c.enc_eps, s))) return rc;
                if ((rc = gemm<EPI_SWIGLU>(eh, He, WE(l, SA_RE_GU_W), He, emlp, c.enc_inter_pad, WE(l, SA_RE_GU_B), nullptr, 0,
                                           Pi, 2 * c.enc_inter_pad, He, s))) return rc;
                if ((rc = gemm<EPI_RESIDUAL>(emlp, c.enc_inter_pad, WE(l, SA_RE_DOWN_W), c.enc_inter_pad, ex, He,
                                             WE(l, SA_RE_DOWN_B), ex, He, Pi, He, c.enc_inter_pad, s))) return rc;
            }
            if ((rc = rmsnorm(ex, He, W(SA_RW_MERGER_LN), eh, He, nullptr, Pi, He, 1e-6f, s))) return rc;
            const int Mg = Pi / unit, Hm = He * unit;
            if ((rc = gemm<EPI_GELU>(eh, Hm, W(SA_RW_FC1_W), Hm, emh, Hm, W(SA_RW_FC1_B), nullptr, 0, Mg, Hm, Hm, s))) return rc;
            if ((rc = gemm<EPI_BIAS>(emh, Hm, W(SA_RW_FC2_W), Hm, emerged, c.enc_out_hidden, W(SA_RW_FC2_B), nullptr, 0, Mg,
                                     c.enc_out_hidden, Hm, s))) return rc;
            hipLaunchKernelGGL(scatter_image_kernel<T>, dim3(Mg), dim3(128), 0, s, emerged, W(SA_RW_IMG_H), W(SA_RW_IMG_W), d_dst,
                               d_hidx, d_widx, dst, c.dec_hidden);
            if ((rc = (int)hipGetLastError())) return rc;
            patch_base += P;
            tok_base += P / unit;
            i0 = i1;
        }
        return SA_OK;
    }

    int encode_only(const float* tiles, const int32_t* grid_hw, int n, void* out, hipStream_t s) override {
        if (c.enc_out_hidden != c.dec_hidden) return SA_ERR_SHAPE;
        long ntok = 0;
        for (int i = 0; i < n; ++i) ntok += (long)grid_hw[2 * i] * grid_hw[2 * i + 1] / (c.merge * c.merge);
        std::vector<int> ident(ntok);
        for (long i = 0; i < ntok; ++i) ident[i] = (int)i;
        return encode(tiles, grid_hw, n, ident, reinterpret_cast<T*>(out), s);
    }

    int encode_ahead(const float* tiles, const int32_t* grid_hw, int n, hipStream_t s) override {
        if (c.enc_out_hidden != c.dec_hidden) return SA_ERR_SHAPE;
        if (n == 0) {
            ahead_consumed = ahead_tokens = 0;
            return SA_OK;
        }
        if (n < 0 || !tiles || !grid_hw) return SA_ERR_ARG;
        if (ahead_consumed != ahead_tokens) return SA_ERR_STATE;
        long ntok = 0;
        for (int i = 0; i < n; ++i) ntok += (long)grid_hw[2 * i] * grid_hw[2 * i + 1] / (c.merge * c.merge);
        if (ntok > std::max(c.max_prefill_tokens, c.max_slots)) return SA_ERR_SHAPE;
        std::vector<int> ident(ntok);
        for (long i = 0; i < ntok; ++i) ident[i] = (int)i;
        SA_HIP(hipEventRecord(ev_ahead_in, s));
        SA_HIP(hipStreamWaitEvent(estream, ev_ahead_in, 0));
        if (ahead_free_recorded) SA_HIP(hipStreamWaitEvent(estream, ev_ahead_free, 0));
        int rc = encode(tiles, grid_hw, n, ident, emb_ahead, estream, st_enc);
        if (rc) return rc;
        SA_HIP(hipEventRecord(ev_ahead_done, estream));
        ahead_tokens = ntok;
        ahead_consumed = 0;
        return SA_OK;
    }

    int decoder_layers_prefill(int M, const int* d_tok_slot, const int* d_tok_pos, const AttnSegs* sg, int n_tiles, hipStream_t s) {
        const int Hd = c.dec_hidden, nq = c.dec_heads, nkv = c.dec_kv_heads, d = c.dec_head_dim, I = c.dec_inter;
        const int qkv_d = (nq + 2 * nkv) * d;
        const float scale = 1.0f / sqrtf((float)d);
        const size_t layer_kv = (size_t)c.max_slots * nkv * c.max_kv_len * d;
        const float* inv_freq = reinterpret_cast<const float*>(w[SA_RW_DEC_INVFREQ]);
        int rc;
        for (int l = 0; l < c.dec_layers; ++l) {
            T* kc = kcache + l * layer_kv;
            T* vc = vcache + l * layer_kv;
            if ((rc = rmsnorm(dx, Hd, WD(l, SA_RD_LN1), dh, Hd, nullptr, M, Hd, c.dec_eps, s))) return rc;
            if ((rc = gemm<EPI_BIAS>(dh, Hd, WD(l, SA_RD_QKV_W), Hd, dqkv, qkv_d, WD(l, SA_RD_QKV_B), nullptr, 0, M, qkv_d, Hd, s)))
                return rc;
            hipLaunchKernelGGL(rope_kv_append_kernel<T>, dim3(M), dim3(256), 0, s, dqkv, d_tok_slot, d_tok_pos, rope_cs, kc, vc,
                               nq, nkv, d, c.max_kv_len);
            if constexpr (std::is_same<T, bf16_t>::value) {
                if (kv8) {
                    const size_t l8 = (size_t)c.max_slots * nkv, T8 = tmax8();
                    uint8_t* k8l = k8c + l * l8 * c.max_kv_len * d;
                    uint8_t* v8l = v8tc + l * l8 * d * T8;
                    float* ksl = ksc8 + l * l8 * T8;
                    float* vsl = vsc8 + l * l8 * T8;
                    dim3 qg(cdiv(M * nkv, 4));
                    if (d == 128) hipLaunchKernelGGL(kv8_quant_rows_kernel<128>, qg, dim3(256), 0, s, kc, vc, d_tok_slot, d_tok_pos, M, k8l, v8l, ksl, vsl, nkv, c.max_kv_len, (int)T8);
                    else if (d == 64) hipLaunchKernelGGL(kv8_quant_rows_kernel<64>, qg, dim3(256), 0, s, kc, vc, d_tok_slot, d_tok_pos, M, k8l, v8l, ksl, vsl, nkv, c.max_kv_len, (int)T8);
                    else if (d == 32) hipLaunchKernelGGL(kv8_quant_rows_kernel<32>, qg, dim3(256), 0, s, kc, vc, d_tok_slot, d_tok_pos, M, k8l, v8l, ksl, vsl, nkv, c.max_kv_len, (int)T8);
                    else return SA_ERR_UNSUPPORTED;
                }
            }
            if ((rc = attention(d, dqkv, kc, vc, dattn, *sg, n_tiles, nq, qkv_d, d, d, (long)c.max_kv_len * d, (long)nq * d, d,
                                nq / nkv, 1, scale, s))) return rc;
            if ((rc = gemm<EPI_RESIDUAL>(dattn, (long)nq * d, WD(l, SA_RD_O_W), (long)nq * d, dx, Hd, nullptr, dx, Hd, M, Hd, nq * d,
                                         s))) return rc;
            if ((rc = rmsnorm(dx, Hd, WD(l, SA_RD_LN2), dh, Hd, nullptr, M, Hd, c.dec_eps, s))) return rc;
            if ((rc = gemm<EPI_SWIGLU>(dh, Hd, WD(l, SA_RD_GU_W), Hd, dmlp, I, nullptr, nullptr, 0, M, 2 * I, Hd, s))) return rc;
            if ((rc = gemm<EPI_RESIDUAL>(dmlp, I, WD(l, SA_RD_DOWN_W), I, dx, Hd, nullptr, dx, Hd, M, Hd, I, s))) return rc;
        }
        return SA_OK;
    }

    struct Half { int r0, M; float* part; hipStream_t s; };

    int splitk_gemm(const T* X, long ldx, const T* Wt, long ldw, int M, int N, int K, float* part_, int* S, hipStream_t s) {
        GemmArgs<T, T> a{X, ldx, Wt, ldw, nullptr, 0, nullptr, nullptr, 0, M, N, K, 1, part_};
        int rc = launch_gemm_splitk<T>(a, s);
        *S = a.splitk;
        return rc;
    }
    int reduce_residual_norm(int S, int M, const float* part_, T* x, const T* wnorm, T* y, hipStream_t s, uint8_t* y8 = nullptr,
                             uint8_t* sy = nullptr, const T* pf_cache = nullptr, const Half* h = nullptr) {
        const int threads = cdiv(c.dec_hidden / 4, 64) * 64;
        if (threads > 1024 || c.dec_hidden % 4) return SA_ERR_UNSUPPORTED;
        KvPrefetch pf;
        if (pf_cache && h && tuning().kvprefetch && (c.dec_head_dim * sizeof(T)) % 16 == 0) {
            pf.base = reinterpret_cast<const unsigned char*>(pf_cache);
            pf.slots = active_dev + h->r0; pf.lens = row_len + h->r0;
            pf.head_stride = (long)c.max_kv_len * c.dec_head_dim * sizeof(T);
            pf.slot_stride = pf.head_stride * c.dec_kv_heads;
            pf.heads = c.dec_kv_heads; pf.row_bytes = c.dec_head_dim * (int)sizeof(T); pf.max_rows = c.max_kv_len;
        }
        const int grid = pf.base ? 2 * M : M;
#define SA_RNORM(SL) hipLaunchKernelGGL((splitk_residual_norm_kernel<T, SL>), dim3(grid), dim3(threads), 0, s, part_, S, M, x, (const T*)nullptr, \
                                        wnorm, y, c.dec_hidden, c.dec_eps, y8, sy, c.max_slots, pf)
        if (tuning().rnorm == 1 || S > 4) SA_RNORM(8);
        else if (S > 2) SA_RNORM(4);
        else SA_RNORM(2);
#undef SA_RNORM
        return (int)hipGetLastError();
    }
    int splitk_gemm_mx(const uint8_t* X, const uint8_t* SX, long ldx, const uint8_t* Wq, const uint8_t* SW, int M, int N, int K,
                       float* part_, int* S, hipStream_t s) {
        MxArgs a{X, ldx, SX, Wq, (long)K, SW, M, N, K, (long)c.max_slots, (long)N};
        a.part = part_;
        int rc = launch_gemm_mx_splitk(a, s);
        *S = a.splitk;
        return rc;
    }

    void drop_graphs() {
        for (auto& kv : graphs) (void)hipGraphExecDestroy(kv.second);
        graphs.clear(); seen_keys.clear();
    }
    int set_kv_fp8(int on) override {
        if constexpr (!std::is_same<T, bf16_t>::value) return on ? SA_ERR_UNSUPPORTED : SA_OK;
        if ((on != 0) != kv8) drop_graphs();
        if (!on) { kv8 = false; return SA_OK; }
        const int d = c.dec_head_dim;
        if (d != 128 && d != 64 && d != 32) return SA_ERR_UNSUPPORTED;
        if (c.dec_heads / c.dec_kv_heads > 8) return SA_ERR_UNSUPPORTED;
        if (!kv8_arena) {
            const size_t rows = (size_t)c.dec_layers * c.max_slots * c.dec_kv_heads, T8 = tmax8();
            size_t off = 0;
            auto take = [&](size_t bytes) { size_t o = off; off = align_up(off + bytes); return o; };
            const size_t o_k = take(rows * c.max_kv_len * d), o_v = take(rows * d * T8), o_ks = take(rows * T8 * 4), o_vs = take(rows * T8 * 4);
            SA_HIP(hipMalloc((void**)&kv8_arena, off));
            SA_HIP(hipMemset(kv8_arena, 0, off));
            SA_HIP(hipDeviceSynchronize());
            k8c = (uint8_t*)(kv8_arena + o_k); v8tc = (uint8_t*)(kv8_arena + o_v);
            ksc8 = (float*)(kv8_arena + o_ks); vsc8 = (float*)(kv8_arena + o_vs);
        }
        kv8 = true;
        return SA_OK;
    }

    int set_mx_weights(const void* const* tbl, int n) override {
        if constexpr (!std::is_same<T, bf16_t>::value) return SA_ERR_UNSUPPORTED;
        if (!tbl) { if (!mxw.empty()) drop_graphs(); mxw.clear(); return SA_OK; }
        if (n != SA_MX_TOTAL(c.dec_layers)) return SA_ERR_ARG;
        for (int i = 0; i < n; ++i)
            if (!tbl[i]) return SA_ERR_ARG;
        const int Hd = c.dec_hidden, A = c.dec_heads * c.dec_head_dim, I = c.dec_inter;
        if (Hd % 128 || A % 128 || I % 128 || c.dec_head_dim % 32) return SA_ERR_SHAPE;
        if (!mx_arena) {
            const size_t S = c.max_slots;
            size_t off = 0;
            auto take = [&](size_t b) { size_t o = off; off = align_up(off + b); return o; };
            const size_t o1 = take(S * Hd), o2 = take(S * Hd / 32), o3 = take(S * A), o4 = take(S * A / 32), o5 = take(S * I),
                         o6 = take(S * I / 32), o7 = take(S * Hd), o8 = take(S * Hd / 32);
            SA_HIP(hipMalloc((void**)&mx_arena, off));
            SA_HIP(hipMemset(mx_arena, 0, off));
// ... 63 lines not shown
    }
#define SA_DEC_MFMA(DD, GG) SA_DEC_LAUNCH((decode_attn_mfma_kernel<T, DD, GG>), (decode_attn_mfma_lds<T, DD, GG>()))
#define SA_DEC_FLASH3(DD, GG) SA_DEC_LAUNCH((decode_attn_flash_kernel<DD, GG>), (decode_attn_flash_lds<DD, GG>()), at8, sat, c.max_slots)
#define SA_DEC_FLASH4(DD, GG)                                                                                                         \
    {                                                                                                                                 \
        const int dbk = tuning().dattn_db;                                                                                            \
        if (dbk == 1 || (dbk == 0 && !tuning().graph && ctx_bound > 128 && M * nkv <= 256))             \
            SA_DEC_LAUNCH((decode_attn_flash2_kernel<DD, GG, true>), (decode_attn_flash2_lds<DD, GG, true>()), at8, sat, c.max_slots) \
        else SA_DEC_LAUNCH((decode_attn_flash2_kernel<DD, GG, false>), (decode_attn_flash2_lds<DD, GG, false>()), at8, sat, c.max_slots) \
    }
#define SA_DEC_FLASH(DD, GG) { if (tuning().dattn == 3) SA_DEC_FLASH3(DD, GG) else SA_DEC_FLASH4(DD, GG) }
        bool launched = false;
        if constexpr (std::is_same<T, bf16_t>::value) {
            if (kv8) {
                const size_t l8 = (size_t)c.max_slots * nkv, T8 = tmax8();
                uint8_t* k8l = k8c + l * l8 * c.max_kv_len * d;
                uint8_t* v8l = v8tc + l * l8 * d * T8;
                float* ksl = ksc8 + l * l8 * T8;
                float* vsl = vsc8 + l * l8 * T8;
#define SA_DEC_KV8(DD, GG)                                                                                                       \
    {                                                                                                                           \
        auto kern = decode_attn_kv8_kernel<DD, GG>;                                                                             \
        static AttrOnce attr;                                                                                                   \
        attr.ensure(kern, decode_attn_kv8_lds<DD, GG>());                                                                       \
        hipLaunchKernelGGL(kern, grid, dim3(KV8_THREADS), (decode_attn_kv8_lds<DD, GG>()), s, h.part, S, WD(l, SA_RD_QKV_B), at, k8l, v8l, ksl, \
                           vsl, act, rl, rope_cs, nq, nkv, c.max_kv_len, (int)T8, scale, at8, sat, c.max_slots);                \
    }
                launched = true;
                if (d == 128 && G <= 5) SA_DEC_KV8(128, 5)
                else if (d == 128 && G <= 8) SA_DEC_KV8(128, 8)
                else if (d == 64 && G <= 8) SA_DEC_KV8(64, 8)
                else if (d == 32 && G <= 8) SA_DEC_KV8(32, 8)
                else return SA_ERR_UNSUPPORTED;
#undef SA_DEC_KV8
            }
        }
        if constexpr (std::is_same<T, bf16_t>::value) {
          if (!launched) {
            launched = true;
            if (d == 128 && G <= 5) SA_DEC_FLASH(128, 5)
            else if (d == 128 && G <= 8) SA_DEC_FLASH(128, 8)
            else if (d == 64 && G <= 8) SA_DEC_FLASH(64, 8)
            else if (d == 32 && G <= 8) SA_DEC_FLASH(32, 8)
            else launched = false;
          }
        }
        if (!launched) {
            if (d == 128 && G <= 5) SA_DEC_MFMA(128, 5)
            else if (d == 128) SA_DEC_MFMA(128, 8)
            else if (d == 64) SA_DEC_MFMA(64, 8)
            else if (d == 32) SA_DEC_MFMA(32, 8)
            else return SA_ERR_UNSUPPORTED;
        }
#undef SA_DEC_FLASH
#undef SA_DEC_FLASH3
#undef SA_DEC_FLASH4
#undef SA_DEC_MFMA
#undef SA_DEC_LAUNCH
        if ((rc = (int)hipGetLastError())) return rc;
        if (q8 && !launched) return SA_ERR_UNSUPPORTED;
        const bool last = (l + 1 == c.dec_layers);
        const T* wnext = last ? W(SA_RW_DEC_NORM) : WD(l + 1, SA_RD_LN1);
        T* ynext = last ? dlast + (size_t)h.r0 * Hd : hh;
        if (q8) {
            if ((rc = splitk_gemm_mx(at8, sat, A, MXW(l, SA_MX_O_W), MXW(l, SA_MX_O_S), M, Hd, A, h.part, &S, s))) return rc;
            if ((rc = reduce_residual_norm(S, M, h.part, x, WD(l, SA_RD_LN2), hh, s, hh8, shh))) return rc;
            MxArgs g{hh8, Hd, shh, MXW(l, SA_MX_GU_W), Hd, MXW(l, SA_MX_GU_S), M, 2 * I, Hd, (long)c.max_slots, (long)2 * I};
            g.Q = ml8; g.ldq = I; g.SQ = sml; g.sq_rows = c.max_slots;
            if ((rc = launch_gemm_mx<MX_EPI_SWIGLU>(g, s))) return rc;
            if ((rc = splitk_gemm_mx(ml8, sml, I, MXW(l, SA_MX_DOWN_W), MXW(l, SA_MX_DOWN_S), M, Hd, I, h.part, &S, s))) return rc;
            return reduce_residual_norm(S, M, h.part, x, wnext, ynext, s, last ? dlast8 + (size_t)h.r0 * Hd : hh8,
                                        last ? slast + (size_t)h.r0 * 4 : shh);
        }
        const bool warm = !last && !kv8;
        const T* v_next = warm ? vcache + (size_t)(l + 1) * layer_kv : nullptr;
        const T* k_next = warm ? kcache + (size_t)(l + 1) * layer_kv : nullptr;
        if ((rc = splitk_gemm(at, (long)nq * d, WD(l, SA_RD_O_W), (long)nq * d, M, Hd, nq * d, h.part, &S, s))) return rc;
        if ((rc = reduce_residual_norm(S, M, h.part, x, WD(l, SA_RD_LN2), hh, s, nullptr, nullptr, v_next, &h))) return rc;
        if ((rc = gemm<EPI_SWIGLU>(hh, Hd, WD(l, SA_RD_GU_W), Hd, ml, I, nullptr, nullptr, 0, M, 2 * I, Hd, s))) return rc;
        if ((rc = splitk_gemm(ml, I, WD(l, SA_RD_DOWN_W), I, M, Hd, I, h.part, &S, s))) return rc;
        return reduce_residual_norm(S, M, h.part, x, wnext, ynext, s, nullptr, nullptr, k_next, &h);
    }

    int heads(int rows, const int* d_last_row, const int* d_row_slot, int step, int len_inc, bool normed, hipStream_t s, bool fuse_next = false) {
        const int Hd = c.dec_hidden;
        int rc;
        T* last = dlast;
        float4* am = amax;
        if (!normed && (rc = rmsnorm(dx, Hd, W(SA_RW_DEC_NORM), last, Hd, d_last_row, rows, Hd, c.dec_eps, s))) return rc;
        int bn_used = 0;
        if (mx() && normed) {
            if constexpr (std::is_same<T, bf16_t>::value) {
                MxArgs a{dlast8, Hd, slast, MXG(SA_MX_LM_W), Hd, MXG(SA_MX_LM_S), rows, c.vocab, Hd, (long)c.max_slots, (long)c.vocab};
                a.amax = am;
                a.bias = W(SA_RW_LM_B);
                if ((rc = launch_gemm_mx<MX_EPI_ARGMAX>(a, s))) return rc;
                bn_used = a.bn_used;
            }
        } else {
            GemmArgs<T, float> a{last, Hd, W(SA_RW_LM_W), Hd, logits, c.vocab, W(SA_RW_LM_B), nullptr, 0, rows, c.vocab, Hd};
            a.amax = am;
            if ((rc = launch_gemm<T, float, EPI_ARGMAX>(a, s))) return rc;
            bn_used = a.bn_used;
        }
        const int tiles_n = cdiv(c.vocab, bn_used);
        const size_t so = (size_t)step * c.max_slots;
        last_rows = rows;
        last_heads_mx = mx() && normed;
        if (head2_ok() && tiles_n <= 4 * SA_HEAD_THREADS) {
            const bool fz = fuse_next;
            hipLaunchKernelGGL((greedy_head2_kernel<T>), dim3(rows), dim3(SA_HEAD_THREADS), 0, s, reinterpret_cast<const float4*>(am), tiles_n,
                               last, Hd, W(SA_RW_BBOX_W), W(SA_RW_BBOX_B), d_row_slot, c.eos_token_id, c.pad_token_id, (float)c.bbox_size,
                               out_token + so, out_score + so, out_bbox + so * 6, next_token, kv_len, len_inc,
                               fz ? W(SA_RW_TOK_EMBED) : (const T*)nullptr, WD(0, SA_RD_LN1), dx, dh, row_len, c.max_kv_len, c.dec_eps,
                               (fz && mx()) ? dh8 : (uint8_t*)nullptr, (fz && mx()) ? sdh : (uint8_t*)nullptr, c.max_slots);
            return (int)hipGetLastError();
        }
        if (fuse_next) return SA_ERR_STATE;
        hipLaunchKernelGGL((greedy_head_kernel<T, true>), dim3(rows), dim3(256), 0, s, reinterpret_cast<const float*>(am),
                           (long)tiles_n, tiles_n, last, Hd, W(SA_RW_BBOX_W), W(SA_RW_BBOX_B), d_row_slot, c.eos_token_id,
                           c.pad_token_id, (float)c.bbox_size, out_token + so, out_score + so, out_bbox + so * 6, next_token,
                           kv_len, len_inc);
        last_rows = rows;
        last_heads_mx = mx() && normed;
        return (int)hipGetLastError();
    }

    int prefill(const float* tiles, const int32_t* grid_hw, int n_images, const int32_t* input_ids, const int32_t* seq_offsets,
                const int32_t* slot_ids, int n_seqs, hipStream_t s) override {
        if (n_seqs <= 0) return SA_OK;
        if (n_seqs > c.max_slots) return SA_ERR_ARG;
        const int Ttot = seq_offsets[n_seqs];
        if (Ttot > c.max_prefill_tokens) return SA_ERR_SHAPE;
        const int nq = c.dec_heads, nkv = c.dec_kv_heads, d = c.dec_head_dim;
        std::vector<int> ids(Ttot), tok_slot(Ttot), tok_pos(Ttot), lens(n_seqs), last_row(n_seqs), img_pos;
        SegLists sg;
        for (int i = 0; i < n_seqs; ++i) {
            const int a = seq_offsets[i], L = seq_offsets[i + 1] - a;
            if (L <= 0 || L >= c.max_kv_len || slot_ids[i] < 0 || slot_ids[i] >= c.max_slots) return SA_ERR_ARG;
            lens[i] = L; last_row[i] = a + L - 1;
            if (h_len.size() < (size_t)c.max_slots) h_len.resize(c.max_slots, 0);
            h_len[slot_ids[i]] = L;
            for (int t = 0; t < L; ++t) {
                const int id = input_ids[a + t];
                if (id < 0 || id >= c.vocab) return SA_ERR_ARG;
                const bool img = (id == c.image_token_id);
                ids[a + t] = img ? -1 : id;
                if (img) img_pos.push_back(a + t);
                tok_slot[a + t] = slot_ids[i]; tok_pos[a + t] = t;
            }
            sg.seg_len.push_back(L);
            sg.q_off.push_back((long)a * (nq + 2 * nkv) * d);
            sg.k_off.push_back((long)slot_ids[i] * nkv * c.max_kv_len * d);
            sg.v_off.push_back((long)slot_ids[i] * nkv * c.max_kv_len * d);
            sg.o_off.push_back((long)a * nq * d);
            sg.add_tiles(i, L);
        }
        long ntok = 0;
        for (int i = 0; i < n_images; ++i) ntok += (long)grid_hw[2 * i] * grid_hw[2 * i + 1] / (c.merge * c.merge);
        if ((long)img_pos.size() != ntok) return SA_ERR_SHAPE;
        int rc;
        st_small.begin();
        const int* d_slots = st_small.put(slot_ids, n_seqs);
        const int* d_lens = st_small.put(lens);
        const int* d_last = st_small.put(last_row);
        if (!d_last) return SA_ERR_NOMEM;
        if ((rc = st_small.flush(s))) return rc;
        {
            st.begin();
            const int* d_ids = st.put(ids);
            if (!d_ids) return SA_ERR_NOMEM;
            if ((rc = st.flush(s))) return rc;
            hipLaunchKernelGGL(embed_tokens_kernel<T>, dim3(Ttot), dim3(128), 0, s, W(SA_RW_TOK_EMBED), d_ids, dx, c.dec_hidden);
        }
        if (n_images > 0 && tiles) {
            if ((rc = encode(tiles, grid_hw, n_images, img_pos, dx, s))) return rc;
        } else if (n_images > 0) {
            if (ahead_consumed + ntok > ahead_tokens) return SA_ERR_STATE;
            st.begin();
            const int* d_img = st.put(img_pos);
            if (!d_img) return SA_ERR_NOMEM;
            if ((rc = st.flush(s))) return rc;
            SA_HIP(hipStreamWaitEvent(s, ev_ahead_done, 0));
            hipLaunchKernelGGL(scatter_rows_kernel<T>, dim3((unsigned)ntok), dim3(128), 0, s, emb_ahead + ahead_consumed * c.dec_hidden,
                               d_img, dx, c.dec_hidden);
            ahead_consumed += ntok;
            SA_HIP(hipEventRecord(ev_ahead_free, s));
            ahead_free_recorded = true;
        }
        st.begin();
        const int* d_tok_slot = st.put(tok_slot);
        const int* d_tok_pos = st.put(tok_pos);
        AttnSegs d_sg = stage_segs(st, sg);
        if (!d_sg.o_off) return SA_ERR_NOMEM;
        if ((rc = st.flush(s))) return rc;
        hipLaunchKernelGGL(set_slot_state_kernel, dim3(cdiv(n_seqs, 256)), dim3(256), 0, s, d_slots, d_lens, kv_len, n_seqs);
        if ((rc = decoder_layers_prefill(Ttot, d_tok_slot, d_tok_pos, &d_sg, (int)sg.tile_seg.size(), s))) return rc;
        return heads(n_seqs, d_last, d_slots, 0, 0, false, s);
    }

    int set_active(const int32_t* slots, int n, hipStream_t s) override {
        if (n < 0 || n > c.max_slots) return SA_ERR_ARG;
        n_active = n;
        for (int i = 0; i < n; ++i)
            if (slots[i] < 0 || slots[i] >= c.max_slots) return SA_ERR_ARG;
        h_active.assign(slots, slots + n);
        if (n == 0) return SA_OK;
        st_small.begin();
        const int* d = st_small.put(slots, n);
        if (!d) return SA_ERR_NOMEM;
        int rc = st_small.flush(s);
        if (rc) return rc;
        SA_HIP(hipMemcpyAsync(active_dev, d, n * sizeof(int), hipMemcpyDeviceToDevice, s));
        return SA_OK;
    }

    bool can_fuse_embed() const {
        return tuning().fuse_embed && head2_ok() && c.dec_hidden <= 2 * 4 * SA_HEAD_THREADS && cdiv(c.vocab, 320) <= 4 * SA_HEAD_THREADS &&
               cdiv(c.vocab, 64) <= 4 * SA_HEAD_THREADS;
    }
    int decode_eager(int M, int n_steps, int step0, hipStream_t s) {
        int rc;
        const Half h{0, M, part, s};
        const bool fuse = can_fuse_embed();
        if (h_len.size() < (size_t)c.max_slots) h_len.resize(c.max_slots, 0);
        for (int step = 0; step < n_steps; ++step) {
            ctx_bound = 0;
            for (int a : h_active) {
                ctx_bound = std::max(ctx_bound, h_len[a] + 1);
                h_len[a] = std::min(h_len[a] + 1, c.max_kv_len);
            }
            if ((step == 0 || !fuse) && (rc = decode_embed(h))) return rc;
            for (int l = 0; l < c.dec_layers; ++l)
                if ((rc = decode_layer(l, h))) return rc;
            if ((rc = heads(M, nullptr, active_dev, step0 + step, 1, true, s, fuse && step + 1 < n_steps))) return rc;
        }
        return SA_OK;
    }

    int decode(int n_steps, hipStream_t s) override { return decode_steps(n_steps, 0, s); }

    int decode_async(int n_steps, int ring, hipStream_t s) override {
        if (n_steps < 0 || n_steps > SA_MAX_STEPS / 2 || ring < 0 || ring > 1) return SA_ERR_ARG;
        int rc = decode_steps(n_steps, ring * (SA_MAX_STEPS / 2), s);
        if (rc) return rc;
        const size_t S = c.max_slots, full = (size_t)SA_MAX_STEPS * S, off = (size_t)ring * (SA_MAX_STEPS / 2) * S;
        const size_t nt = (size_t)n_steps * S;
        if (nt) {
            SA_HIP(hipMemcpyAsync(out_host + off * 4, out_token + off, nt * sizeof(int), hipMemcpyDeviceToHost, s));
            SA_HIP(hipMemcpyAsync(out_host + full * 4 + off * 4, out_score + off, nt * sizeof(float), hipMemcpyDeviceToHost, s));
            SA_HIP(hipMemcpyAsync(out_host + full * 8 + off * 24, out_bbox + off * 6, nt * 6 * sizeof(int), hipMemcpyDeviceToHost, s));
        }
        SA_HIP(hipEventRecord(ev_ring[ring], s));
        return SA_OK;
    }

    int wait_outputs(int n_steps, int ring, int32_t* tokens, float* scores, int32_t* bboxes) override {
        if (n_steps < 0 || n_steps > SA_MAX_STEPS / 2 || ring < 0 || ring > 1) return SA_ERR_ARG;
        SA_HIP(hipEventSynchronize(ev_ring[ring]));
        const size_t S = c.max_slots, full = (size_t)SA_MAX_STEPS * S, off = (size_t)ring * (SA_MAX_STEPS / 2) * S;
        const size_t nt = (size_t)n_steps * S;
        memcpy(tokens, out_host + off * 4, nt * sizeof(int));
        memcpy(scores, out_host + full * 4 + off * 4, nt * sizeof(float));
        memcpy(bboxes, out_host + full * 8 + off * 24, nt * 6 * sizeof(int));
        return SA_OK;
    }

    int decode_steps(int n_steps, int step0, hipStream_t s) {
        if (n_steps < 0 || step0 < 0 || step0 + n_steps > SA_MAX_STEPS) return SA_ERR_ARG;
        const int M = n_active;
        if (M == 0 || n_steps == 0) return SA_OK;
        if (!use_graph || !tuning().graph || gemm_profiler().enabled) return decode_eager(M, n_steps, step0, s);
        if (graph_epoch != tuning_epoch()) { drop_graphs(); graph_epoch = tuning_epoch(); }
        const long key = ((long)M * 64 + n_steps) * 64 + step0;
        auto it = graphs.find(key);
        if (it == graphs.end()) {
            if (!seen_keys.count(key)) { seen_keys.insert(key); return decode_eager(M, n_steps, step0, s); }
            hipGraph_t g = nullptr;
            SA_HIP(hipStreamBeginCapture(gstream, hipStreamCaptureModeThreadLocal));
            int rc = decode_eager(M, n_steps, step0, gstream);
            hipError_t e = hipStreamEndCapture(gstream, &g);
            if (rc || e != hipSuccess || !g) {
                if (g) (void)hipGraphDestroy(g);
                (void)hipGetLastError();
                use_graph = false;
                return decode_eager(M, n_steps, step0, s);
            }
            hipGraphExec_t ex = nullptr;
            e = hipGraphInstantiate(&ex, g, nullptr, nullptr, 0);
            (void)hipGraphDestroy(g);
            if (e != hipSuccess) { use_graph = false; (void)hipGetLastError(); return decode_eager(M, n_steps, step0, s); }
            it = graphs.emplace(key, ex).first;
        }
        SA_HIP(hipEventRecord(gev_in, s));
        SA_HIP(hipStreamWaitEvent(gstream, gev_in, 0));
        SA_HIP(hipGraphLaunch(it->second, gstream));
        SA_HIP(hipEventRecord(gev_out, gstream));
        SA_HIP(hipStreamWaitEvent(s, gev_out, 0));
        return SA_OK;
    }

    int read_outputs(int n_steps, int32_t* tokens, float* scores, int32_t* bboxes, hipStream_t s) override {
        if (n_steps <= 0 || n_steps > SA_MAX_STEPS) return SA_ERR_ARG;
        const size_t S = c.max_slots, full = (size_t)SA_MAX_STEPS * S;
        const size_t nt = (size_t)n_steps * S;
        SA_HIP(hipMemcpyAsync(out_host, out_token, nt * sizeof(int), hipMemcpyDeviceToHost, s));
        SA_HIP(hipMemcpyAsync(out_host + full * 4, out_score, nt * sizeof(float), hipMemcpyDeviceToHost, s));
        SA_HIP(hipMemcpyAsync(out_host + full * 8, out_bbox, nt * 6 * sizeof(int), hipMemcpyDeviceToHost, s));
        SA_HIP(hipStreamSynchronize(s));
        memcpy(tokens, out_host, nt * sizeof(int));
        memcpy(scores, out_host + full * 4, nt * sizeof(float));
        memcpy(bboxes, out_host + full * 8, nt * 6 * sizeof(int));
        return SA_OK;
    }

    int copy_last_logits(float* dst, int max_rows, int* rows, hipStream_t s) override {
        const int r = std::min(max_rows, last_rows);
        *rows = r;
        if (r <= 0) return SA_OK;
        const int Hd = c.dec_hidden;
        int rc;
        if (last_heads_mx) {
            if constexpr (std::is_same<T, bf16_t>::value) {
                MxArgs a{dlast8, Hd, slast, MXG(SA_MX_LM_W), Hd, MXG(SA_MX_LM_S), last_rows, c.vocab, Hd, (long)c.max_slots, (long)c.vocab};
                a.C = logits; a.ldc = c.vocab; a.bias = W(SA_RW_LM_B);
                if ((rc = launch_gemm_mx<MX_EPI_F32>(a, s))) return rc;
            }
        } else {
            GemmArgs<T, float> a{dlast, Hd, W(SA_RW_LM_W), Hd, logits, c.vocab, W(SA_RW_LM_B), nullptr, 0, last_rows, c.vocab, Hd};
            if ((rc = launch_gemm<T, float, EPI_BIAS>(a, s))) return rc;
        }
        SA_HIP(hipMemcpyAsync(dst, logits, (size_t)r * c.vocab * sizeof(float), hipMemcpyDeviceToDevice, s));
        return SA_OK;
    }

    int set_next_tokens(const int32_t* slots, const int32_t* toks, int n, hipStream_t s) override {
        if (n <= 0) return SA_OK;
        st_small.begin();
        const int* ds = st_small.put(slots, n);
        const int* dt = st_small.put(toks, n);
        if (!dt) return SA_ERR_NOMEM;
        int rc = st_small.flush(s);
        if (rc) return rc;
        hipLaunchKernelGGL(set_next_tokens_kernel, dim3(cdiv(n, 256)), dim3(256), 0, s, ds, dt, next_token, n);
        return (int)hipGetLastError();
    }
};

static int check_cfg(const surya_rec_config* c) {
    if (!c) return SA_ERR_ARG;
    if (c->dtype != SA_DTYPE_F32 && c->dtype != SA_DTYPE_BF16) return SA_ERR_UNSUPPORTED;
    if (c->enc_hidden % 64 || c->enc_inter_pad % 64 || c->patch_dim_pad % 64 || c->dec_hidden % 64 || c->dec_inter % 64 ||
        (c->dec_heads * c->dec_head_dim) % 64 || c->vocab % 4)
        return SA_ERR_SHAPE;
    if (c->enc_hidden % c->enc_heads || c->dec_heads % c->dec_kv_heads || c->dec_heads / c->dec_kv_heads > 8) return SA_ERR_SHAPE;
    if (c->merge != 2 || c->window_tokens <= 0 || c->enc_depth > 32) return SA_ERR_UNSUPPORTED;
    if (c->max_slots <= 0 || c->max_kv_len <= 0 || c->max_patches < 4 || c->max_prefill_tokens <= 0) return SA_ERR_ARG;
    return SA_OK;
}

}

using namespace sa;
struct surya_rec { std::unique_ptr<RecBase> impl; surya_rec_config cfg; };

namespace sa {
int op_gemm_f16(int epi, const void* X, long ldx, const void* W, long ldw, void* C, long ldc, const void* bias, const void* R, long ldr,
                int M, int N, int K, hipStream_t s);
}
template <typename TI, typename TO>
static int op_gemm_t(int epi, const void* X, long ldx, const void* W, long ldw, void* C, long ldc, const void* bias, const void* R,
                     long ldr, int M, int N, int K, hipStream_t s) {
    GemmArgs<TI, TO> a{(const TI*)X, ldx, (const TI*)W, ldw, (TO*)C, ldc, (const TI*)bias, (const TO*)R, ldr, M, N, K};
    switch (epi) {
        case EPI_BIAS: return launch_gemm<TI, TO, EPI_BIAS>(a, s);
        case EPI_RESIDUAL: return R ? launch_gemm<TI, TO, EPI_RESIDUAL>(a, s) : SA_ERR_ARG;
        case EPI_GELU: return launch_gemm<TI, TO, EPI_GELU>(a, s);
        case EPI_SWIGLU: return launch_gemm<TI, TO, EPI_SWIGLU>(a, s);
        case EPI_HARDSWISH: return launch_gemm<TI, TO, EPI_HARDSWISH>(a, s);
        case EPI_RELU: return launch_gemm<TI, TO, EPI_RELU>(a, s);
    }
    return SA_ERR_ARG;
}


extern "C" {

const char* surya_amd_version(void) { return "surya_amd 0.1.0 gfx950"; }

size_t surya_rec_workspace_bytes(const surya_rec_config* cfg) {
    if (check_cfg(cfg)) return 0;
    return cfg->dtype == SA_DTYPE_F32 ? RecModel<float>::layout(*cfg, nullptr) : RecModel<bf16_t>::layout(*cfg, nullptr);
}

int surya_rec_create(const surya_rec_config* cfg, const void* const* weights, int n_weights, surya_rec** out) {
    int rc = check_cfg(cfg);
    if (rc) return rc;
    if (!weights || !out || n_weights != SA_RW_TOTAL(cfg->enc_depth, cfg->dec_layers)) return SA_ERR_ARG;
    for (int i = 0; i < n_weights; ++i)
        if (!weights[i]) return SA_ERR_ARG;
    auto* h = new surya_rec();
    h->cfg = *cfg;
    if (cfg->dtype == SA_DTYPE_F32) {
        auto m = std::make_unique<RecModel<float>>();
        rc = m->init(*cfg, weights, n_weights);
        h->impl = std::move(m);
    } else {
        auto m = std::make_unique<RecModel<bf16_t>>();
        rc = m->init(*cfg, weights, n_weights);
        h->impl = std::move(m);
    }
    if (rc) { delete h; return rc; }
    *out = h;
    return SA_OK;
}

int surya_rec_destroy(surya_rec* h) {
    if (!h) return SA_ERR_ARG;
    (void)hipDeviceSynchronize();
    delete h;
    return SA_OK;
}

int surya_rec_plan_encoder(const surya_rec_config* cfg, const int32_t* grid_hw, int n_images, int32_t* src_row, int32_t* pos_hw,
                           int32_t* cu_window, int32_t* n_windows, int32_t* merged_src) {
    if (!cfg || !grid_hw || n_images <= 0) return SA_ERR_ARG;
    EncPlan pl;
    int rc = plan_encoder(*cfg, grid_hw, n_images, pl);
    if (rc) return rc;
    if (src_row) memcpy(src_row, pl.src_row.data(), pl.src_row.size() * sizeof(int));
    if (pos_hw) memcpy(pos_hw, pl.pos_hw.data(), pl.pos_hw.size() * sizeof(int));
    if (cu_window) memcpy(cu_window, pl.win_cu.data(), pl.win_cu.size() * sizeof(int));
    if (n_windows) *n_windows = (int)pl.win_cu.size() - 1;
    if (merged_src) memcpy(merged_src, pl.merged_src.data(), pl.merged_src.size() * sizeof(int));
    return SA_OK;
}

int surya_rec_prefill(surya_rec* h, const float* tiles, const int32_t* grid_hw, int n_images, const int32_t* input_ids,
                      const int32_t* seq_offsets, const int32_t* slot_ids, int n_seqs, void* stream) {
    if (!h || !input_ids || !seq_offsets || !slot_ids || (n_images > 0 && !grid_hw)) return SA_ERR_ARG;
    return h->impl->prefill(tiles, grid_hw, n_images, input_ids, seq_offsets, slot_ids, n_seqs, (hipStream_t)stream);
}
int surya_rec_encode_ahead(surya_rec* h, const float* tiles, const int32_t* grid_hw, int n_images, void* stream) {
    if (!h || n_images < 0 || (n_images > 0 && (!tiles || !grid_hw))) return SA_ERR_ARG;
    return h->impl->encode_ahead(tiles, grid_hw, n_images, (hipStream_t)stream);
}
int surya_rec_set_active(surya_rec* h, const int32_t* slots, int n_active, void* stream) {
    if (!h || (n_active > 0 && !slots)) return SA_ERR_ARG;
    return h->impl->set_active(slots, n_active, (hipStream_t)stream);
}
int surya_rec_decode(surya_rec* h, int n_steps, void* stream) {
    if (!h) return SA_ERR_ARG;
    return h->impl->decode(n_steps, (hipStream_t)stream);
}
int surya_rec_read_outputs(surya_rec* h, int n_steps, int32_t* tokens, float* scores, int32_t* bboxes, void* stream) {
    if (!h || !tokens || !scores || !bboxes) return SA_ERR_ARG;
    return h->impl->read_outputs(n_steps, tokens, scores, bboxes, (hipStream_t)stream);
}
int surya_rec_decode_async(surya_rec* h, int n_steps, int ring, void* stream) {
    if (!h) return SA_ERR_ARG;
    return h->impl->decode_async(n_steps, ring, (hipStream_t)stream);
}
int surya_rec_wait_outputs(surya_rec* h, int n_steps, int ring, int32_t* tokens, float* scores, int32_t* bboxes) {
    if (!h || !tokens || !scores || !bboxes) return SA_ERR_ARG;
    return h->impl->wait_outputs(n_steps, ring, tokens, scores, bboxes);
}
int surya_rec_encode_only(surya_rec* h, const float* tiles, const int32_t* grid_hw, int n_images, void* out, void* stream) {
    if (!h || !tiles || !grid_hw || !out || n_images <= 0) return SA_ERR_ARG;
    return h->impl->encode_only(tiles, grid_hw, n_images, out, (hipStream_t)stream);
}
int surya_rec_copy_last_logits(surya_rec* h, float* dst, int max_rows, int* rows, void* stream) {
    if (!h || !dst || !rows || max_rows <= 0) return SA_ERR_ARG;
    return h->impl->copy_last_logits(dst, max_rows, rows, (hipStream_t)stream);
}
int surya_rec_set_next_tokens(surya_rec* h, const int32_t* slots, const int32_t* tokens, int n, void* stream) {
    if (!h || !slots || !tokens) return SA_ERR_ARG;
    return h->impl->set_next_tokens(slots, tokens, n, (hipStream_t)stream);
}

int surya_rec_set_mx_weights(surya_rec* h, const void* const* table, int n) {
    if (!h) return SA_ERR_ARG;
    return h->impl->set_mx_weights(table, n);
}

int surya_rec_set_kv_fp8(surya_rec* h, int on) {
    if (!h) return SA_ERR_ARG;
    return h->impl->set_kv_fp8(on);
}

int surya_op_gemm(int dtype, int out_f32, int epi, const void* X, long ldx, const void* W, long ldw, void* C, long ldc,
                  const void* bias, const void* R, long ldr, int M, int N, int K, void* stream) {
    if (!X || !W || !C) return SA_ERR_ARG;
    hipStream_t s = (hipStream_t)stream;
    if (dtype == SA_DTYPE_F32) return op_gemm_t<float, float>(epi, X, ldx, W, ldw, C, ldc, bias, R, ldr, M, N, K, s);
    if (dtype == SA_DTYPE_BF16)
        return out_f32 ? op_gemm_t<bf16_t, float>(epi, X, ldx, W, ldw, C, ldc, bias, R, ldr, M, N, K, s)
                       : op_gemm_t<bf16_t, bf16_t>(epi, X, ldx, W, ldw, C, ldc, bias, R, ldr, M, N, K, s);
    if (dtype == SA_DTYPE_F16)
        return out_f32 ? SA_ERR_UNSUPPORTED : sa::op_gemm_f16(epi, X, ldx, W, ldw, C, ldc, bias, R, ldr, M, N, K, s);
    return SA_ERR_UNSUPPORTED;
}

namespace {
struct DevSegs {
    void* mem = nullptr;
    sa::AttnSegs a{};
    int n_tiles = 0;
    int init(const int32_t* seg_len, const int64_t* q_off, const int64_t* k_off, const int64_t* v_off, const int64_t* o_off, int n_seg) {
        std::vector<int> tile_seg, tile_q0;
        for (int s = 0; s < n_seg; ++s) {
            if (seg_len[s] <= 0) return SA_ERR_ARG;
            for (int q0 = 0; q0 < seg_len[s]; q0 += 64) { tile_seg.push_back(s); tile_q0.push_back(q0); }
        }
        n_tiles = (int)tile_seg.size();
        const size_t ib = ((size_t)(2 * n_tiles + n_seg) * sizeof(int) + 15) & ~(size_t)15, lb = (size_t)n_seg * sizeof(long);
        std::vector<char> host(ib + 4 * lb);
        int* hi = reinterpret_cast<int*>(host.data());
        memcpy(hi, tile_seg.data(), n_tiles * sizeof(int));
        memcpy(hi + n_tiles, tile_q0.data(), n_tiles * sizeof(int));
        memcpy(hi + 2 * n_tiles, seg_len, n_seg * sizeof(int));
        const int64_t* offs[4] = {q_off, k_off, v_off, o_off};
        for (int i = 0; i < 4; ++i) memcpy(host.data() + ib + i * lb, offs[i], lb);
        SA_HIP(hipMalloc(&mem, host.size()));
        SA_HIP(hipMemcpy(mem, host.data(), host.size(), hipMemcpyHostToDevice));
        char* d = reinterpret_cast<char*>(mem);
        a.tile_seg = reinterpret_cast<const int*>(d); a.tile_q0 = a.tile_seg + n_tiles; a.seg_len = a.tile_seg + 2 * n_tiles;
        a.q_off = reinterpret_cast<const long*>(d + ib); a.k_off = a.q_off + n_seg; a.v_off = a.q_off + 2 * n_seg; a.o_off = a.q_off + 3 * n_seg;
        return SA_OK;
    }
    ~DevSegs() { if (mem) (void)hipFree(mem); }
};
}

int surya_op_attn(int dtype, int head_dim, const void* q, const void* k, const void* v, void* out, const int32_t* seg_len,
                  const int64_t* q_off, const int64_t* k_off, const int64_t* v_off, const int64_t* o_off, int n_seg, int heads, int group,
                  int causal, float scale, long q_row, long q_head, long k_row, long k_head, long o_row, long o_head, void* stream) {
    if (!q || !k || !v || !out || !seg_len || !q_off || !k_off || !v_off || !o_off || n_seg <= 0 || heads <= 0 || group <= 0) return SA_ERR_ARG;
    hipStream_t s = (hipStream_t)stream;
    DevSegs sg;
    int rc = sg.init(seg_len, q_off, k_off, v_off, o_off, n_seg);
    if (rc) return rc;
    dim3 grid(sg.n_tiles, heads);
#define SA_OPA_M(DD) hipLaunchKernelGGL((attn_mfma_kernel<DD>), grid, dim3(128), 0, s, (const bf16_t*)q, (const bf16_t*)k, (const bf16_t*)v, \
                                        (bf16_t*)out, sg.a, q_row, q_head, k_row, k_head, o_row, o_head, group, causal, scale)
#define SA_OPA_V(DD) hipLaunchKernelGGL((attn_valu_kernel<float, DD>), grid, dim3(256), 0, s, (const float*)q, (const float*)k, (const float*)v, \
                                        (float*)out, sg.a, q_row, q_head, k_row, k_head, o_row, o_head, group, causal, scale)
    if (dtype == SA_DTYPE_BF16) {
        switch (head_dim) {
            case 32: SA_OPA_M(32); break;
            case 64: SA_OPA_M(64); break;
            case 80: SA_OPA_M(80); break;
            case 128: SA_OPA_M(128); break;
            default: return SA_ERR_UNSUPPORTED;
        }
    } else if (dtype == SA_DTYPE_F32) {
        switch (head_dim) {
            case 32: SA_OPA_V(32); break;
            case 64: SA_OPA_V(64); break;
            case 80: SA_OPA_V(80); break;
            case 128: SA_OPA_V(128); break;
            default: return SA_ERR_UNSUPPORTED;
        }
    } else {
        return SA_ERR_UNSUPPORTED;
    }
#undef SA_OPA_M
#undef SA_OPA_V
    SA_HIP(hipGetLastError());
    SA_HIP(hipStreamSynchronize(s));
    return SA_OK;
}

int surya_op_decode_attn(int dtype, int head_dim, const float* qkv_part, int n_slabs, const void* qkv_bias, void* out, void* kcache,
                         void* vcache, const int32_t* active_slots, const int32_t* row_len, const float* rope_cs, int rows, int heads,
                         int kv_heads, int max_kv_len, float scale, void* stream) {
    if (!qkv_part || !qkv_bias || !out || !kcache || !vcache || !active_slots || !row_len || !rope_cs) return SA_ERR_ARG;
    if (rows <= 0 || n_slabs < 1 || n_slabs > 8 || kv_heads <= 0 || heads % kv_heads) return SA_ERR_ARG;
    hipStream_t s = (hipStream_t)stream;
    const int G = heads / kv_heads, d = head_dim;
    dim3 grid(rows, kv_heads), block(256);
    const float2* cs = reinterpret_cast<const float2*>(rope_cs);
#define SA_OPD(KERN, LDS, TT, ...)                                                                                              \
    {                                                                                                                           \
        auto kern = KERN;                                                                                                       \
        static AttrOnce attr;                                                                                                   \
        attr.ensure(kern, LDS);                                                                                                 \
        hipLaunchKernelGGL(kern, grid, block, LDS, s, qkv_part, n_slabs, (const TT*)qkv_bias, (TT*)out, (TT*)kcache, (TT*)vcache, \
                           active_slots, row_len, cs, heads, kv_heads, max_kv_len, scale, ##__VA_ARGS__);                       \
    }
#define SA_OPD_FLASH3(DD, GG) SA_OPD((decode_attn_flash_kernel<DD, GG>), (decode_attn_flash_lds<DD, GG>()), bf16_t, (uint8_t*)nullptr, (uint8_t*)nullptr, 0)
#define SA_OPD_FLASH4(DD, GG)                                                                                                                 \
    {                          \
        if (tuning().dattn_db == 1)                                                                                                           \
            SA_OPD((decode_attn_flash2_kernel<DD, GG, true>), (decode_attn_flash2_lds<DD, GG, true>()), bf16_t, (uint8_t*)nullptr, (uint8_t*)nullptr, 0) \
        else SA_OPD((decode_attn_flash2_kernel<DD, GG, false>), (decode_attn_flash2_lds<DD, GG, false>()), bf16_t, (uint8_t*)nullptr, (uint8_t*)nullptr, 0) \
    }
#define SA_OPD_FLASH(DD, GG) { if (tuning().dattn == 3) SA_OPD_FLASH3(DD, GG) else SA_OPD_FLASH4(DD, GG) }
#define SA_OPD_MFMA(DD, GG) SA_OPD((decode_attn_mfma_kernel<float, DD, GG>), (decode_attn_mfma_lds<float, DD, GG>()), float)
    if (dtype == SA_DTYPE_BF16) {
        if (d == 128 && G <= 5) SA_OPD_FLASH(128, 5)
        else if (d == 128 && G <= 8) SA_OPD_FLASH(128, 8)
        else if (d == 64 && G <= 8) SA_OPD_FLASH(64, 8)
        else if (d == 32 && G <= 8) SA_OPD_FLASH(32, 8)
        else return SA_ERR_UNSUPPORTED;
    } else if (dtype == SA_DTYPE_F32) {
        if (d == 128 && G <= 5) SA_OPD_MFMA(128, 5)
        else if (d == 128 && G <= 8) SA_OPD_MFMA(128, 8)
        else if (d == 64 && G <= 8) SA_OPD_MFMA(64, 8)
        else if (d == 32 && G <= 8) SA_OPD_MFMA(32, 8)
        else return SA_ERR_UNSUPPORTED;
    } else {
        return SA_ERR_UNSUPPORTED;
    }
#undef SA_OPD_FLASH
#undef SA_OPD_FLASH3
#undef SA_OPD_FLASH4
#undef SA_OPD_MFMA
#undef SA_OPD
    return (int)hipGetLastError();
}

int surya_op_kv8_quant_rows(int head_dim, const void* kcache, const void* vcache, const int32_t* tok_slot, const int32_t* tok_pos, int n_tokens,
                            void* k8, void* v8t, float* kscale, float* vscale, int kv_heads, int max_kv_len, void* stream) {
    if (!kcache || !vcache || !tok_slot || !tok_pos || !k8 || !v8t || !kscale || !vscale || n_tokens <= 0 || kv_heads <= 0) return SA_ERR_ARG;
    hipStream_t s = (hipStream_t)stream;
    const int T8 = (max_kv_len + 255) & ~255;
    dim3 qg(cdiv(n_tokens * kv_heads, 4));
#define SA_Q8(DD)                                                                                                                  \
    hipLaunchKernelGGL(kv8_quant_rows_kernel<DD>, qg, dim3(256), 0, s, (const bf16_t*)kcache, (const bf16_t*)vcache, tok_slot, tok_pos, \
                       n_tokens, (uint8_t*)k8, (uint8_t*)v8t, kscale, vscale, kv_heads, max_kv_len, T8)
    if (head_dim == 128) SA_Q8(128);
    else if (head_dim == 64) SA_Q8(64);
    else if (head_dim == 32) SA_Q8(32);
    else return SA_ERR_UNSUPPORTED;
#undef SA_Q8
    return (int)hipGetLastError();
}

int surya_op_decode_attn_kv8(int head_dim, const float* qkv_part, int n_slabs, const void* qkv_bias, void* out, void* k8, void* v8t,
                             float* kscale, float* vscale, const int32_t* active_slots, const int32_t* row_len, const float* rope_cs, int rows,
                             int heads, int kv_heads, int max_kv_len, float scale, void* stream) {
    if (!qkv_part || !qkv_bias || !out || !k8 || !v8t || !kscale || !vscale || !active_slots || !row_len || !rope_cs) return SA_ERR_ARG;
    if (rows <= 0 || n_slabs < 1 || n_slabs > 8 || kv_heads <= 0 || heads % kv_heads) return SA_ERR_ARG;
    hipStream_t s = (hipStream_t)stream;
    const int G = heads / kv_heads, d = head_dim, T8 = (max_kv_len + 255) & ~255;
    dim3 grid(rows, kv_heads), block(256);
    const float2* cs = reinterpret_cast<const float2*>(rope_cs);
#define SA_OPD8(DD, GG)                                                                                                          \
    {                                                                                                                           \
        auto kern = decode_attn_kv8_kernel<DD, GG>;                                                                             \
// ... 5 lines not shown
    }
    if (d == 128 && G <= 5) SA_OPD8(128, 5)
    else if (d == 128 && G <= 8) SA_OPD8(128, 8)
    else if (d == 64 && G <= 8) SA_OPD8(64, 8)
    else if (d == 32 && G <= 8) SA_OPD8(32, 8)
    else return SA_ERR_UNSUPPORTED;
#undef SA_OPD8
    return (int)hipGetLastError();
}

__global__ __launch_bounds__(256) void mx_quantize_rows_kernel(const float* __restrict__ x, int K, uint8_t* __restrict__ q,
                                                               uint8_t* __restrict__ sc) {
    const long row = blockIdx.x, rows = gridDim.x;
    for (int c = threadIdx.x * 4; c < K; c += 1024) {
        float v[4];
        load4(x + row * K + c, v);
        int e8;
        const uint32_t pk = mx_quant4_oct(v, e8);
        *reinterpret_cast<uint32_t*>(q + row * K + c) = pk;
        if ((threadIdx.x & 7) == 0) sc[((long)(c >> 7) * rows + row) * 4 + ((c >> 5) & 3)] = (uint8_t)e8;
    }
}

int surya_op_mx_quantize(const float* x, int rows, int K, uint8_t* q, uint8_t* scales, void* stream) {
    if (!x || !q || !scales || rows <= 0 || K <= 0 || K % 128) return SA_ERR_ARG;
    hipLaunchKernelGGL(mx_quantize_rows_kernel, dim3(rows), dim3(256), 0, (hipStream_t)stream, x, K, q, scales);
    return (int)hipGetLastError();
}

int surya_op_gemm_splitk_bf16(const void* X, long ldx, const void* W, long ldw, float* part, int M, int N, int K, int* splitk, void* stream) {
    if (!X || !W || !part || !splitk) return SA_ERR_ARG;
    GemmArgs<bf16_t, bf16_t> a{reinterpret_cast<const bf16_t*>(X), ldx, reinterpret_cast<const bf16_t*>(W), ldw, nullptr, 0, nullptr, nullptr, 0, M, N, K, 1, part};
    const int rc = launch_gemm_splitk<bf16_t>(a, (hipStream_t)stream);
    *splitk = a.splitk;
    return rc;
}

int surya_op_gemm_mx(int mode, const uint8_t* X, const uint8_t* SX, const uint8_t* W, const uint8_t* SW, int M, int N, int K,
                     float* C, int* splitk, uint8_t* q_out, uint8_t* sq_out, void* stream) {
    if (!X || !SX || !W || !SW) return SA_ERR_ARG;
    MxArgs a{X, (long)K, SX, W, (long)K, SW, M, N, K, (long)M, (long)N};
    hipStream_t s = (hipStream_t)stream;
    if (mode == 0) {
        if (!C) return SA_ERR_ARG;
        a.C = C; a.ldc = N;
        return launch_gemm_mx<MX_EPI_F32>(a, s);
    }
    if (mode == 1) {
        if (!C || !splitk) return SA_ERR_ARG;
        a.part = C;
        int rc = launch_gemm_mx_splitk(a, s);
        *splitk = a.splitk;
        return rc;
    }
    if (mode == 2) {
        if (!q_out || !sq_out) return SA_ERR_ARG;
        a.Q = q_out; a.ldq = N / 2; a.SQ = sq_out; a.sq_rows = M;
        return launch_gemm_mx<MX_EPI_SWIGLU>(a, s);
    }
    return SA_ERR_ARG;
}

int surya_rec_preprocess(const uint8_t* pages, const void* lines, int n_lines, uint8_t* mask_arena, float* mid_arena, float* tiles,
                         int patch_size, int merge_size, float pad_value, const float* mean, const float* std, int any_poly,
                         int max_stage1_width, int pixel_stride, void* stream) {
    if (!pages || !lines || !tiles || !mean || !std || n_lines < 0 || patch_size <= 0 || merge_size <= 0) return SA_ERR_ARG;
    if (pixel_stride != 3 && pixel_stride != 4) return SA_ERR_ARG;
    sa::prep::PrepArgs p;
    p.pages = pages; p.lines = reinterpret_cast<const sa::prep::LineDesc*>(lines); p.n_lines = n_lines;
    p.mask = mask_arena; p.mid = mid_arena; p.tiles = tiles; p.ps = patch_size; p.merge = merge_size; p.pad = pad_value;
    for (int i = 0; i < 3; ++i) { p.mean[i] = mean[i]; p.std[i] = std[i]; }
    p.max_mid_w = max_stage1_width;
    p.pix = pixel_stride;
    return sa::prep::prep_run(p, any_poly, max_stage1_width > 0, (hipStream_t)stream);
}

int surya_set_tuning(const char* key, int value) {
    if (!key) return SA_ERR_ARG;
    Tuning& t = tuning();
    struct { const char* k; int* v; } tab[] = {
        {"graph", &t.graph}, {"split_target", &t.split_target}, {"split_min_kt", &t.split_min_kt}, {"split_max", &t.split_max},
        {"bigtile", &t.bigtile}, {"bigtile_any", &t.bigtile_any}, {"conv_lean", &t.conv_lean}, {"conv_persist", &t.conv_persist}, {"dwconv_pipe", &t.dwconv_pipe}, {"bigtile_ratio_pct", &t.bigtile_ratio_pct}, {"gateup_ring", &t.gateup_ring}, {"dring", &t.dring}, {"dring_min_kt", &t.dring_min_kt}, {"big_m_split", &t.big_m_split}, {"big_m_gateup", &t.big_m_gateup}, {"glds", &t.glds}, {"bigtile_min_k", &t.bigtile_min_k}, {"dattn", &t.dattn}, {"rnorm", &t.rnorm},
        {"ghead", &t.ghead}, {"fuse_embed", &t.fuse_embed}, {"persist", &t.persist}, {"lmhead", &t.lmhead}, {"kvprefetch", &t.kvprefetch},
        {"dattn_db", &t.dattn_db}, {"lay_ln", &t.lay_ln}, {"det_head_blk", &t.det_head_blk}, {"det_fuse", &t.det_fuse}, {"det_up4", &t.det_up4}, {"fmb_chunk", &t.fmb_chunk}, {"ocrerr_cls_only", &t.ocrerr_cls_only}};
    for (auto& e : tab)
        if (!strcmp(e.k, key)) {
            if (*e.v != value) ++tuning_epoch();
            *e.v = value;
            return SA_OK;
        }
    return SA_ERR_ARG;
}

int surya_gemm_ring_status(int reset) { return sa::ring_error(reset != 0); }

int surya_prof_enable(int on) {
    GemmProfiler& pf = gemm_profiler();
    if (on) pf.start(); else pf.enabled = false;
    return SA_OK;
}

__global__ void prof_null_kernel() {}

int surya_prof_event_overhead(void* stream, double* ms) {
    if (!ms) return SA_ERR_ARG;
    hipStream_t s = (hipStream_t)stream;
    constexpr int N = 201;
    hipEvent_t ev[2 * N];
    for (auto& e : ev) SA_HIP(hipEventCreate(&e));
    for (int i = 0; i < 32; ++i) hipLaunchKernelGGL(prof_null_kernel, dim3(1), dim3(64), 0, s);
    for (int i = 0; i < N; ++i) {
        SA_HIP(hipEventRecord(ev[2 * i], s));
        hipLaunchKernelGGL(prof_null_kernel, dim3(1), dim3(64), 0, s);
        SA_HIP(hipEventRecord(ev[2 * i + 1], s));
    }
    SA_HIP(hipStreamSynchronize(s));
    std::vector<float> t(N);
    for (int i = 0; i < N; ++i) SA_HIP(hipEventElapsedTime(&t[i], ev[2 * i], ev[2 * i + 1]));
    for (auto& e : ev) (void)hipEventDestroy(e);
    std::sort(t.begin(), t.end());
    *ms = t[N / 2];
    return SA_OK;
}

int surya_prof_read2(int max_cfg, int* launches, double* ms, double* flops, double* bytes, double* slab_bytes) {
    GemmProfiler& pf = gemm_profiler();
    if (!launches || !ms || !flops || !bytes || max_cfg < GemmProfiler::NCFG) return SA_ERR_ARG;
    SA_HIP(hipDeviceSynchronize());
    for (int c = 0; c < GemmProfiler::NCFG; ++c) { launches[c] = 0; ms[c] = flops[c] = bytes[c] = 0.0; if (slab_bytes) slab_bytes[c] = 0.0; }
    for (int i = 0; i < pf.n; ++i) {
        float t = 0.f;
        SA_HIP(hipEventElapsedTime(&t, pf.ev[2 * i], pf.ev[2 * i + 1]));
        const int c = pf.cfg_of[i];
        launches[c]++; ms[c] += t; flops[c] += pf.flops_of[i]; bytes[c] += pf.bytes_of[i];
        if (slab_bytes) slab_bytes[c] += pf.slab_of[i];
    }
    pf.n = 0;
    return SA_OK;
}

int surya_prof_read(int max_cfg, int* launches, double* ms, double* flops, double* bytes) {
    return surya_prof_read2(max_cfg, launches, ms, flops, bytes, nullptr);
}

int surya_op_rmsnorm(int dtype, const void* x, long ldx, const void* w, void* y, long ldy, int rows, int C, float eps,
                     void* stream) {
    if (!x || !w || !y || rows <= 0) return SA_ERR_ARG;
    hipStream_t s = (hipStream_t)stream;
    if (dtype == SA_DTYPE_F32)
        hipLaunchKernelGGL(rmsnorm_kernel<float>, dim3(cdiv(rows, 4)), dim3(256), 0, s, (const float*)x, ldx, (const float*)w,
                           (float*)y, ldy, (const int*)nullptr, rows, C, eps);
    else if (dtype == SA_DTYPE_BF16)
        hipLaunchKernelGGL(rmsnorm_kernel<bf16_t>, dim3(cdiv(rows, 4)), dim3(256), 0, s, (const bf16_t*)x, ldx, (const bf16_t*)w,
                           (bf16_t*)y, ldy, (const int*)nullptr, rows, C, eps);
    else
        return SA_ERR_UNSUPPORTED;
    return (int)hipGetLastError();
}

}
```

### surya_amd/recognition/model.py

```python
from __future__ import annotations

import ctypes as C
from typing import List, Optional, Sequence

import numpy as np
import torch

from .. import _lib as L
from ..config import RecConfig
from .weights import repack_rec_weights, pad64


class HipRecModel:
    def __init__(self, cfg: RecConfig, state_dict, *, image_token_id: int, pad_token_id: int, eos_token_id: int,
                 dtype: torch.dtype = torch.bfloat16, device="cuda:0", max_slots: int = 256, max_kv_len: int = 512,
                 max_patches: int = 65536, max_prefill_tokens: Optional[int] = None, broadcast_weights: bool = False,
                 process_group=None, decode_fp8: Optional[bool] = None):
        if not torch.cuda.is_available():
            raise L.SuryaAmdError("HipRecModel needs a GPU (MI355X); there is no CPU fallback")
        self.lib = L.lib()
        self.cfg = cfg
        self.device = torch.device(device)
        self.dtype = dtype
        torch.cuda.set_device(self.device)
# ... 77 lines not shown

    def to(self, device_dtype=None):
        if device_dtype is None:
            return self
        want_dev, want_dt = None, None
        if isinstance(device_dtype, torch.dtype):
            want_dt = device_dtype
        else:
            want_dev = torch.device("cuda:0" if device_dtype == "cuda" else device_dtype)
        if (want_dt is not None and want_dt != self.dtype) or (want_dev is not None and want_dev != self.device):
            raise NotImplementedError(f"HipRecModel lives on {self.device} as {self.dtype}; create a new predictor for "
                                      f"{device_dtype} (the HIP handle owns device memory; there is no CPU path)")
        return self

    def eval(self):
        return self

    @property
    def _stream(self):
        return C.c_void_p(torch.cuda.current_stream(self.device).cuda_stream)

    def prefill(self, tiles: torch.Tensor, grid_hw, input_ids: Sequence[Sequence[int]], slot_ids: Sequence[int]):
        torch.cuda.set_device(self.device)
        grid = np.ascontiguousarray(np.asarray(grid_hw, np.int32).reshape(-1, 2))
        offs = np.zeros(len(input_ids) + 1, np.int32)
        offs[1:] = np.cumsum([len(s) for s in input_ids])
        flat = np.ascontiguousarray(np.concatenate([np.asarray(s, np.int32) for s in input_ids]))
        slots = np.ascontiguousarray(np.asarray(slot_ids, np.int32))
        if tiles is not None:
            assert tiles.is_cuda and tiles.dtype == torch.float32 and tiles.is_contiguous()
            assert tiles.shape[0] == int((grid[:, 0] * grid[:, 1]).sum()) and tiles.shape[1] == self.cfg.encoder.patch_dim
        L.check(self.lib.surya_rec_prefill(self.handle, L.ptr(tiles), L.np_ptr(grid), C.c_int(len(grid)), L.np_ptr(flat),
                                           L.np_ptr(offs), L.np_ptr(slots), C.c_int(len(slots)), self._stream),
                "surya_rec_prefill")

    def encode_ahead(self, tiles: torch.Tensor, grid_hw):
        torch.cuda.set_device(self.device)
        grid = np.ascontiguousarray(np.asarray(grid_hw, np.int32).reshape(-1, 2))
        assert tiles.is_cuda and tiles.dtype == torch.float32 and tiles.is_contiguous()
        assert tiles.shape[0] == int((grid[:, 0] * grid[:, 1]).sum()) and tiles.shape[1] == self.cfg.encoder.patch_dim
        L.check(self.lib.surya_rec_encode_ahead(self.handle, L.ptr(tiles), L.np_ptr(grid), C.c_int(len(grid)), self._stream),
                "surya_rec_encode_ahead")

    def discard_ahead(self):
        L.check(self.lib.surya_rec_encode_ahead(self.handle, None, None, C.c_int(0), self._stream), "surya_rec_encode_ahead(discard)")

    def set_active(self, slots: Sequence[int]):
        a = np.ascontiguousarray(np.asarray(slots, np.int32))
        L.check(self.lib.surya_rec_set_active(self.handle, L.np_ptr(a), C.c_int(len(a)), self._stream), "surya_rec_set_active")

    def decode(self, n_steps: int = 1):
        L.check(self.lib.surya_rec_decode(self.handle, C.c_int(n_steps), self._stream), "surya_rec_decode")

    def read_outputs(self, n_steps: int = 1):
        L.check(self.lib.surya_rec_read_outputs(self.handle, C.c_int(n_steps), L.np_ptr(self._tok),
                                                L.np_ptr(self._score, C.c_float), L.np_ptr(self._bbox), self._stream),
                "surya_rec_read_outputs")
        return self._tok[:n_steps], self._score[:n_steps], self._bbox[:n_steps]

    def decode_async(self, n_steps: int, ring: int):
        L.check(self.lib.surya_rec_decode_async(self.handle, C.c_int(n_steps), C.c_int(ring), self._stream), "surya_rec_decode_async")

    def wait_outputs(self, n_steps: int, ring: int):
        h = L.SA_MAX_STEPS // 2
        tok, sc, bb = self._tok[ring * h:], self._score[ring * h:], self._bbox[ring * h:]
        L.check(self.lib.surya_rec_wait_outputs(self.handle, C.c_int(n_steps), C.c_int(ring), L.np_ptr(tok), L.np_ptr(sc, C.c_float),
                                                L.np_ptr(bb)), "surya_rec_wait_outputs")
        return tok[:n_steps], sc[:n_steps], bb[:n_steps]

    def set_next_tokens(self, slots, tokens):
        s = np.ascontiguousarray(np.asarray(slots, np.int32))
        t = np.ascontiguousarray(np.asarray(tokens, np.int32))
        L.check(self.lib.surya_rec_set_next_tokens(self.handle, L.np_ptr(s), L.np_ptr(t), C.c_int(len(s)), self._stream),
                "surya_rec_set_next_tokens")

    def encode_only(self, tiles: torch.Tensor, grid_hw) -> torch.Tensor:
        grid = np.ascontiguousarray(np.asarray(grid_hw, np.int32).reshape(-1, 2))
        ntok = int((grid[:, 0] * grid[:, 1]).sum()) // (self.cfg.encoder.spatial_merge_size ** 2)
        out = torch.empty((ntok, self.cfg.decoder.hidden_size), dtype=self.dtype, device=self.device)
        L.check(self.lib.surya_rec_encode_only(self.handle, L.ptr(tiles), L.np_ptr(grid), C.c_int(len(grid)), L.ptr(out),
                                               self._stream), "surya_rec_encode_only")
        return out

    def last_logits(self) -> torch.Tensor:
        buf = torch.empty((self.max_slots, self.vocab), dtype=torch.float32, device=self.device)
        rows = C.c_int(0)
        L.check(self.lib.surya_rec_copy_last_logits(self.handle, L.ptr(buf), C.c_int(self.max_slots), C.byref(rows),
                                                    self._stream), "surya_rec_copy_last_logits")
        return buf[: rows.value]
```

Measured before the change: 3247 lines/s.

## Fuse prefill RoPE/KV append into QKV GEMM, last-row-only final layer, occupancy attention

Adds a GEMM epilogue that applies RoPE and writes K/V straight into the cache during prefill, removing the separate rope_kv_append pass and the round trip through the QKV buffer. The final decoder layer now computes attention and the rest of the layer only for each sequence's last row, since only those rows feed the heads. Encoder attention for head dims 80 and 128 uses a variant with a fixed waves-per-EU attribute to control occupancy. It also adds a KV-row copy API for debugging. These paths bring new indexing complexity, and the rope arithmetic is rewritten with explicit fma, which may change rounding slightly.

Measured after the change: 3284 lines/s, median of 6. 1.1% higher.

```diff
diff --git a/include/surya_amd.h b/include/surya_amd.h
--- a/include/surya_amd.h
+++ b/include/surya_amd.h
@@ -82,6 +82,7 @@
 
 int surya_rec_encode_only(surya_rec* h, const float* tiles, const int32_t* grid_hw, int n_images, void* out, void* stream);
 int surya_rec_copy_last_logits(surya_rec* h, float* dst, int max_rows, int* rows, void* stream);
+int surya_rec_copy_kv_rows(surya_rec* h, int layer, int slot, int rows, void* k_out, void* v_out, void* stream);
 int surya_rec_set_next_tokens(surya_rec* h, const int32_t* slots, const int32_t* tokens, int n, void* stream);
 
 enum { SA_MX_QKV_W = 0, SA_MX_QKV_S, SA_MX_O_W, SA_MX_O_S, SA_MX_GU_W, SA_MX_GU_S, SA_MX_DOWN_W, SA_MX_DOWN_S, SA_MX_COUNT };
diff --git a/surya_amd/csrc/attn_mfma.h b/surya_amd/csrc/attn_mfma.h
--- a/surya_amd/csrc/attn_mfma.h
+++ b/surya_amd/csrc/attn_mfma.h
@@ -7,10 +7,10 @@
 typedef short s16x4 __attribute__((ext_vector_type(4)));
 
 template <int D>
-__global__ __launch_bounds__(128) void attn_mfma_kernel(const bf16_t* __restrict__ q, const bf16_t* __restrict__ k,
-                                                        const bf16_t* __restrict__ v, bf16_t* __restrict__ out, AttnSegs sg,
-                                                        long q_row, long q_head, long k_row, long k_head, long o_row, long o_head,
-                                                        int group, int causal, float scale) {
+__device__ __forceinline__ void attn_mfma_body(const bf16_t* __restrict__ q, const bf16_t* __restrict__ k,
+                                               const bf16_t* __restrict__ v, bf16_t* __restrict__ out, const AttnSegs& sg,
+                                               long q_row, long q_head, long k_row, long k_head, long o_row, long o_head,
+                                               int group, int causal, float scale) {
     static_assert(D % 16 == 0 && D <= 128, "head dim");
     constexpr int KC = 64;
     constexpr int PK = D + 8;
@@ -153,4 +153,20 @@
     }
 }
 
+template <int D>
+__global__ __launch_bounds__(128) void attn_mfma_kernel(const bf16_t* __restrict__ q, const bf16_t* __restrict__ k,
+                                                        const bf16_t* __restrict__ v, bf16_t* __restrict__ out, AttnSegs sg,
+                                                        long q_row, long q_head, long k_row, long k_head, long o_row, long o_head,
+                                                        int group, int causal, float scale) {
+    attn_mfma_body<D>(q, k, v, out, sg, q_row, q_head, k_row, k_head, o_row, o_head, group, causal, scale);
 }
+
+template <int D, int W>
+__global__ __launch_bounds__(128) __attribute__((amdgpu_waves_per_eu(W, W)))
+void attn_mfma_occ_kernel(const bf16_t* __restrict__ q, const bf16_t* __restrict__ k, const bf16_t* __restrict__ v, bf16_t* __restrict__ out,
+                          AttnSegs sg, long q_row, long q_head, long k_row, long k_head, long o_row, long o_head, int group, int causal,
+                          float scale) {
+    attn_mfma_body<D>(q, k, v, out, sg, q_row, q_head, k_row, k_head, o_row, o_head, group, causal, scale);
+}
+
+}
diff --git a/surya_amd/csrc/common.h b/surya_amd/csrc/common.h
--- a/surya_amd/csrc/common.h
+++ b/surya_amd/csrc/common.h
@@ -250,6 +250,9 @@
     int fmb_chunk = 64;
     int persist = 1;
     int ocrerr_cls_only = 1;
+    int prefill_last_only = 1;
+    int enc_attn = 2;
+    int prefill_rope_epi = 1;
 };
 inline Tuning& tuning() { static Tuning t; return t; }
 inline int& tuning_epoch() { static int e = 0; return e; }
diff --git a/surya_amd/csrc/gemm.h b/surya_amd/csrc/gemm.h
--- a/surya_amd/csrc/gemm.h
+++ b/surya_amd/csrc/gemm.h
@@ -9,7 +9,8 @@
 namespace sa {
 
 enum GemmEpi { EPI_BIAS = 0, EPI_RESIDUAL = 1, EPI_GELU = 2, EPI_SWIGLU = 3, EPI_HARDSWISH = 4, EPI_RELU = 5, EPI_ARGMAX = 6, EPI_ROPE = 7,
-               EPI_GEGLU = 8  };
+               EPI_GEGLU = 8 ,
+               EPI_ROPE_KV = 9  };
 
 template <typename TI, typename TO>
 struct GemmArgs {
@@ -34,6 +35,11 @@
     FastDiv fd_hw, fd_wo;
     unsigned cv_m1 = 0, cv_m2 = 0;
     int cv_rowskip = 0;
+    const int* tok_slot = nullptr;
+    const int* tok_pos = nullptr;
+    TO* kc = nullptr;
+    TO* vc = nullptr;
+    int kv_nq = 0, kv_nkv = 0, kv_tmax = 0;
 #ifndef SA_P8_TIMING
 #define SA_P8_TIMING 0
 #endif
@@ -1055,8 +1061,66 @@
         using Pk = typename std::conditional<GLU, unsigned, u32x2>::type;
         const unsigned bpack = bpack_raw & bias_mask;
         Pk pk[4][2][4];
-#pragma unroll
-        for (int jp = 0; jp < 2; ++jp)
+        [[maybe_unused]] int kv_head = 0;
+        [[maybe_unused]] unsigned kv_rowoff[2] = {0u, 0u};
+        if constexpr (EPI == EPI_ROPE_KV) {
+            kv_head = __builtin_amdgcn_readfirstlane((n0 + wn * 128) >> 7);
+            int kv_pos[2];
+#pragma unroll
+            for (int i = 0; i < 2; ++i) {
+                const int m = min(m0 + wm * 64 + i * 32 + srow, p.M - 1);
+                kv_pos[i] = p.tok_pos[m];
+                kv_rowoff[i] = (unsigned)p.tok_slot[m];
+            }
+#pragma unroll
+            for (int i = 0; i < 2; ++i) kv_rowoff[i] = ((kv_rowoff[i] * (unsigned)p.kv_nkv * (unsigned)p.kv_tmax + (unsigned)kv_pos[i]) * 128u) * (unsigned)sizeof(TO);
+            if (kv_head < p.kv_nq + p.kv_nkv) {
+#pragma unroll
+                for (int i = 0; i < 2; ++i)
+#pragma unroll
+                    for (int jl = 0; jl < 2; ++jl) {
+                        float4 cs4[4][2];
+#pragma unroll
+                        for (int g = 0; g < 4; ++g) {
+                            const float4* tp = reinterpret_cast<const float4*>(p.rope + (long)kv_pos[i] * 64 + (jl * 32 + g * 8 + lhi * 4));
+                            cs4[g][0] = tp[0]; cs4[g][1] = tp[1];
+                        }
+#pragma unroll
+                        for (int g = 0; g < 4; ++g) {
+                            const int wc = jl * 32 + g * 8 + lhi * 4;
+                            const unsigned lo1 = (unsigned)__builtin_amdgcn_ds_bpermute((wc >> 1) << 2, (int)bpack), hi1 = (unsigned)__builtin_amdgcn_ds_bpermute(((wc >> 1) + 1) << 2, (int)bpack);
+                            const unsigned lo2 = (unsigned)__builtin_amdgcn_ds_bpermute(((wc >> 1) + 32) << 2, (int)bpack), hi2 = (unsigned)__builtin_amdgcn_ds_bpermute(((wc >> 1) + 33) << 2, (int)bpack);
+                            const float b1[4] = {H16<TI>::lo(lo1), H16<TI>::hi(lo1), H16<TI>::lo(hi1), H16<TI>::hi(hi1)};
+                            const float b2[4] = {H16<TI>::lo(lo2), H16<TI>::hi(lo2), H16<TI>::lo(hi2), H16<TI>::hi(hi2)};
+                            const float cs[4] = {cs4[g][0].x, cs4[g][0].z, cs4[g][1].x, cs4[g][1].z};
+                            const float sn[4] = {cs4[g][0].y, cs4[g][0].w, cs4[g][1].y, cs4[g][1].w};
+                            float y1[4], y2[4];
+#pragma unroll
+                            for (int r = 0; r < 4; ++r) {
+                                const float x1 = Ty<TO>::rnd(acc[jl][i][4 * g + r] + b1[r]), x2 = Ty<TO>::rnd(acc[jl + 2][i][4 * g + r] + b2[r]);
+                                y1[r] = __fmaf_rn(x1, cs[r], -__fmul_rn(x2, sn[r]));
+                                y2[r] = __fmaf_rn(x1, sn[r], __fmul_rn(x2, cs[r]));
+                            }
+                            pk[jl][i][g] = Pk{H16<TO>::pk(y1[0], y1[1]), H16<TO>::pk(y1[2], y1[3])};
+                            pk[jl + 2][i][g] = Pk{H16<TO>::pk(y2[0], y2[1]), H16<TO>::pk(y2[2], y2[3])};
+                        }
+                    }
+            } else {
+#pragma unroll
+                for (int j = 0; j < 4; ++j)
+#pragma unroll
+                    for (int i = 0; i < 2; ++i)
+#pragma unroll
+                        for (int g = 0; g < 4; ++g) {
+                            const int wc = j * 32 + g * 8 + lhi * 4;
+                            const unsigned lo = (unsigned)__builtin_amdgcn_ds_bpermute((wc >> 1) << 2, (int)bpack), hi = (unsigned)__builtin_amdgcn_ds_bpermute(((wc >> 1) + 1) << 2, (int)bpack);
+                            pk[j][i][g] = Pk{H16<TO>::pk(acc[j][i][4 * g] + H16<TI>::lo(lo), acc[j][i][4 * g + 1] + H16<TI>::hi(lo)),
+                                             H16<TO>::pk(acc[j][i][4 * g + 2] + H16<TI>::lo(hi), acc[j][i][4 * g + 3] + H16<TI>::hi(hi))};
+                        }
+            }
+        }
+#pragma unroll
+        for (int jp = 0; jp < (EPI == EPI_ROPE_KV ? 0 : 2); ++jp)
 #pragma unroll
             for (int i = 0; i < 2; ++i) {
                 [[maybe_unused]] float4 rope_v[2][4];
@@ -1148,6 +1212,17 @@
 #pragma unroll
             for (int it = 0; it < 4; ++it) {
                 const int rl = wm * 64 + i * 32 + it * 8 + rrow;
+                if constexpr (EPI == EPI_ROPE_KV) {
+                    const unsigned ro = (unsigned)__builtin_amdgcn_ds_bpermute((it * 8 + rrow) << 2, (int)kv_rowoff[i]);
+                    if (kv_head >= p.kv_nq) {
+                        if (rl >= rows_left || cl >= cols_left) continue;
+                        const bool isk = kv_head < p.kv_nq + p.kv_nkv;
+                        unsigned char* base = reinterpret_cast<unsigned char*>(isk ? p.kc : p.vc);
+                        const unsigned ho = (unsigned)((kv_head - p.kv_nq - (isk ? 0 : p.kv_nkv)) * p.kv_tmax * 128 + jh * 64 + rc * 8) * (unsigned)sizeof(TO);
+                        *reinterpret_cast<u32x4*>(base + ho + ro) = raw[it];
+                        continue;
+                    }
+                }
                 if (rl >= rows_left || cl >= cols_left) continue;
                 TO* dst = reinterpret_cast<TO*>(c_tile + (unsigned)(rl * (int)(p.ldc * sizeof(TO)) + cl * (int)sizeof(TO)));
                 if constexpr (EPI == EPI_RESIDUAL) {
@@ -1289,6 +1364,19 @@
 #include "gemm_ring.h"
 namespace sa {
 
+template <typename TI, typename TO>
+static inline bool rope_kv_takes_persist(const GemmArgs<TI, TO>& a) {
+    if constexpr (sizeof(TI) != 2 || sizeof(TO) != 2) return false;
+    const Tuning& t = tuning();
+    if (a.M <= 256 || a.rope_D != 128 || a.N != (a.kv_nq + 2 * a.kv_nkv) * 128 || a.K % Ty<TI>::KE != 0 || a.ldc % 8 != 0) return false;
+    const int nk = a.K / Ty<TI>::KE;
+    const long big = (long)cdiv(a.M, 128) * cdiv(a.N, 128), t256 = (long)cdiv(a.M, 256) * cdiv(a.N, 256);
+    const double ratio256 = t.bigtile_ratio_pct > 0 ? t.bigtile_ratio_pct / 100.0 : (t.bigtile == 3 ? 1.4 : 1.17);
+    const double cost256 = (double)cdivl(t256, 256) * 256 * 4 / ratio256, cost128 = (double)cdivl(big, 512) * 512;
+    return t.bigtile && a.K >= t.bigtile_min_k && ((t256 >= 256 && cost256 <= cost128) || t.bigtile_any) && t.persist && nk >= 4 && nk % 2 == 0 &&
+           a.N % 8 == 0;
+}
+
 template <typename TI, typename TO, int EPI>
 static inline int launch_gemm(const GemmArgs<TI, TO>& a, hipStream_t s) {
     if (a.M <= 0 || a.N <= 0) return SA_OK;
diff --git a/surya_amd/csrc/kernels.h b/surya_amd/csrc/kernels.h
--- a/surya_amd/csrc/kernels.h
+++ b/surya_amd/csrc/kernels.h
@@ -177,6 +177,17 @@
 }
 
 template <typename T>
+__global__ void gather_rows2_kernel(const T* __restrict__ src_a, T* __restrict__ dst_a, int Ha, const T* __restrict__ src_b,
+                                    T* __restrict__ dst_b, int Hb, const int* __restrict__ src_row) {
+    const int r = blockIdx.x;
+    const int H = blockIdx.y ? Hb : Ha;
+    const T* s = (blockIdx.y ? src_b : src_a) + (long)src_row[r] * H;
+    T* d = (blockIdx.y ? dst_b : dst_a) + (long)r * H;
+    for (int c = threadIdx.x * Ty<T>::V16; c < H; c += blockDim.x * Ty<T>::V16)
+        *reinterpret_cast<uint4*>(d + c) = *reinterpret_cast<const uint4*>(s + c);
+}
+
+template <typename T>
 __global__ void scatter_image_kernel(const T* __restrict__ merged, const T* __restrict__ hemb, const T* __restrict__ wemb,
                                      const int* __restrict__ dst_row, const int* __restrict__ hidx, const int* __restrict__ widx,
                                      T* __restrict__ embeds, int H) {
@@ -227,7 +238,7 @@
         const float cs = csn.x, sn = csn.y;
         T* v = row + (long)hh * D;
         const float x1 = Ty<T>::ld(v + i), x2 = Ty<T>::ld(v + i + half);
-        const float y1 = x1 * cs - x2 * sn, y2 = x2 * cs + x1 * sn;
+        const float y1 = __fmaf_rn(x1, cs, -__fmul_rn(x2, sn)), y2 = __fmaf_rn(x1, sn, __fmul_rn(x2, cs));
         if (hh < nq) {
             Ty<T>::st(v + i, y1); Ty<T>::st(v + i + half, y2);
         } else {
diff --git a/surya_amd/csrc/rec_model.hip b/surya_amd/csrc/rec_model.hip
--- a/surya_amd/csrc/rec_model.hip
+++ b/surya_amd/csrc/rec_model.hip
@@ -139,6 +139,7 @@
     virtual int wait_outputs(int, int, int32_t*, float*, int32_t*) = 0;
     virtual int encode_only(const float*, const int32_t*, int, void*, hipStream_t) = 0;
     virtual int copy_last_logits(float*, int, int*, hipStream_t) = 0;
+    virtual int copy_kv_rows(int, int, int, void*, void*, hipStream_t) = 0;
     virtual int set_next_tokens(const int32_t*, const int32_t*, int, hipStream_t) = 0;
     virtual int set_mx_weights(const void* const*, int) = 0;
     virtual int set_kv_fp8(int) = 0;
@@ -322,9 +323,14 @@
         dim3 grid(n_tiles, heads), block(256);
         if constexpr (std::is_same<T, bf16_t>::value) {
             {
-#define SA_ATTN_M(DD)                                                                                                    \
-    hipLaunchKernelGGL((attn_mfma_kernel<DD>), grid, dim3(128), 0, s, q, k, v, o, sg, q_row, q_head, k_row, k_head, o_row, \
-                       o_head, group, causal, scale)
+#define SA_ATTN_K(KERN)                                                                                                  \
+    hipLaunchKernelGGL(KERN, grid, dim3(128), 0, s, q, k, v, o, sg, q_row, q_head, k_row, k_head, o_row, o_head, group, causal, scale)
+#define SA_ATTN_M(DD) SA_ATTN_K((attn_mfma_kernel<DD>))
+                const int occ = tuning().enc_attn;
+                if (occ == 2 && (D == 80 || D == 128)) {
+                    if (D == 80) SA_ATTN_K((attn_mfma_occ_kernel<80, 2>)); else SA_ATTN_K((attn_mfma_occ_kernel<128, 2>));
+                    return (int)hipGetLastError();
+                }
                 switch (D) {
                     case 32: SA_ATTN_M(32); break;
                     case 64: SA_ATTN_M(64); break;
@@ -333,6 +339,7 @@
                     default: return SA_ERR_UNSUPPORTED;
                 }
 #undef SA_ATTN_M
+#undef SA_ATTN_K
                 return (int)hipGetLastError();
             }
         }
@@ -474,7 +481,9 @@
         return SA_OK;
     }
 
-    int decoder_layers_prefill(int M, const int* d_tok_slot, const int* d_tok_pos, const AttnSegs* sg, int n_tiles, hipStream_t s) {
+    int decoder_layers_prefill(int M, const int* d_tok_slot, const int* d_tok_pos, const AttnSegs* sg, int n_tiles, hipStream_t s,
+                               const AttnSegs* sg_last = nullptr, int n_last_tiles = 0, const int* d_last_row = nullptr, int n_seqs = 0,
+                               const T** head_src = nullptr) {
         const int Hd = c.dec_hidden, nq = c.dec_heads, nkv = c.dec_kv_heads, d = c.dec_head_dim, I = c.dec_inter;
         const int qkv_d = (nq + 2 * nkv) * d;
         const float scale = 1.0f / sqrtf((float)d);
@@ -485,10 +494,20 @@
             T* kc = kcache + l * layer_kv;
             T* vc = vcache + l * layer_kv;
             if ((rc = rmsnorm(dx, Hd, WD(l, SA_RD_LN1), dh, Hd, nullptr, M, Hd, c.dec_eps, s))) return rc;
-            if ((rc = gemm<EPI_BIAS>(dh, Hd, WD(l, SA_RD_QKV_W), Hd, dqkv, qkv_d, WD(l, SA_RD_QKV_B), nullptr, 0, M, qkv_d, Hd, s)))
-                return rc;
-            hipLaunchKernelGGL(rope_kv_append_kernel<T>, dim3(M), dim3(256), 0, s, dqkv, d_tok_slot, d_tok_pos, rope_cs, kc, vc,
-                               nq, nkv, d, c.max_kv_len);
+            GemmArgs<T, T> qa{dh, Hd, WD(l, SA_RD_QKV_W), Hd, dqkv, qkv_d, WD(l, SA_RD_QKV_B), nullptr, 0, M, qkv_d, Hd};
+            qa.rope = rope_cs; qa.rope_D = d; qa.tok_slot = d_tok_slot; qa.tok_pos = d_tok_pos; qa.kc = kc; qa.vc = vc;
+            qa.kv_nq = nq; qa.kv_nkv = nkv; qa.kv_tmax = c.max_kv_len;
+            bool fused = false;
+            if constexpr (std::is_same<T, bf16_t>::value)
+                fused = tuning().prefill_rope_epi && !kv8 && layer_kv * sizeof(T) < ((size_t)1 << 32) && rope_kv_takes_persist(qa);
+            if (fused) {
+                if constexpr (std::is_same<T, bf16_t>::value)
+                    if ((rc = launch_gemm_persist<T, T, EPI_ROPE_KV>(qa, s))) return rc;
+            } else {
+                if ((rc = launch_gemm<T, T, EPI_BIAS>(qa, s))) return rc;
+                hipLaunchKernelGGL(rope_kv_append_kernel<T>, dim3(M), dim3(256), 0, s, dqkv, d_tok_slot, d_tok_pos, rope_cs, kc, vc,
+                                   nq, nkv, d, c.max_kv_len);
+            }
             if constexpr (std::is_same<T, bf16_t>::value) {
                 if (kv8) {
                     const size_t l8 = (size_t)c.max_slots * nkv, T8 = tmax8();
@@ -503,6 +522,23 @@
                     else return SA_ERR_UNSUPPORTED;
                 }
             }
+            if (sg_last && l == c.dec_layers - 1) {
+                const size_t slab = (size_t)c.max_slots * std::max(qkv_d, Hd);
+                T* cx = reinterpret_cast<T*>(part);
+                T* cattn = reinterpret_cast<T*>(part + slab);
+                const int R = n_seqs;
+                if ((rc = attention(d, dqkv, kc, vc, dattn, *sg_last, n_last_tiles, nq, qkv_d, d, d, (long)c.max_kv_len * d, (long)nq * d,
+                                    d, nq / nkv, 1, scale, s))) return rc;
+                hipLaunchKernelGGL(gather_rows2_kernel<T>, dim3(R, 2), dim3(128), 0, s, dx, cx, Hd, dattn, cattn, nq * d, d_last_row);
+                if ((rc = (int)hipGetLastError())) return rc;
+                if ((rc = gemm<EPI_RESIDUAL>(cattn, (long)nq * d, WD(l, SA_RD_O_W), (long)nq * d, cx, Hd, nullptr, cx, Hd, R, Hd, nq * d,
+                                             s))) return rc;
+                if ((rc = rmsnorm(cx, Hd, WD(l, SA_RD_LN2), dh, Hd, nullptr, R, Hd, c.dec_eps, s))) return rc;
+                if ((rc = gemm<EPI_SWIGLU>(dh, Hd, WD(l, SA_RD_GU_W), Hd, dmlp, I, nullptr, nullptr, 0, R, 2 * I, Hd, s))) return rc;
+                if ((rc = gemm<EPI_RESIDUAL>(dmlp, I, WD(l, SA_RD_DOWN_W), I, cx, Hd, nullptr, cx, Hd, R, Hd, I, s))) return rc;
+                *head_src = cx;
+                return SA_OK;
+            }
             if ((rc = attention(d, dqkv, kc, vc, dattn, *sg, n_tiles, nq, qkv_d, d, d, (long)c.max_kv_len * d, (long)nq * d, d,
                                 nq / nkv, 1, scale, s))) return rc;
             if ((rc = gemm<EPI_RESIDUAL>(dattn, (long)nq * d, WD(l, SA_RD_O_W), (long)nq * d, dx, Hd, nullptr, dx, Hd, M, Hd, nq * d,
@@ -511,6 +547,7 @@
             if ((rc = gemm<EPI_SWIGLU>(dh, Hd, WD(l, SA_RD_GU_W), Hd, dmlp, I, nullptr, nullptr, 0, M, 2 * I, Hd, s))) return rc;
             if ((rc = gemm<EPI_RESIDUAL>(dmlp, I, WD(l, SA_RD_DOWN_W), I, dx, Hd, nullptr, dx, Hd, M, Hd, I, s))) return rc;
         }
+        if (head_src) *head_src = dx;
         return SA_OK;
     }
 
@@ -740,12 +777,12 @@
         return reduce_residual_norm(S, M, h.part, x, wnext, ynext, s, nullptr, nullptr, k_next, &h);
     }
 
-    int heads(int rows, const int* d_last_row, const int* d_row_slot, int step, int len_inc, bool normed, hipStream_t s, bool fuse_next = false) {
+    int heads(int rows, const T* src, const int* d_last_row, const int* d_row_slot, int step, int len_inc, bool normed, hipStream_t s, bool fuse_next = false) {
         const int Hd = c.dec_hidden;
         int rc;
         T* last = dlast;
         float4* am = amax;
-        if (!normed && (rc = rmsnorm(dx, Hd, W(SA_RW_DEC_NORM), last, Hd, d_last_row, rows, Hd, c.dec_eps, s))) return rc;
+        if (!normed && (rc = rmsnorm(src, Hd, W(SA_RW_DEC_NORM), last, Hd, d_last_row, rows, Hd, c.dec_eps, s))) return rc;
         int bn_used = 0;
         if (mx() && normed) {
             if constexpr (std::is_same<T, bf16_t>::value) {
@@ -851,10 +888,20 @@
         const int* d_tok_pos = st.put(tok_pos);
         AttnSegs d_sg = stage_segs(st, sg);
         if (!d_sg.o_off) return SA_ERR_NOMEM;
+        const bool last_only = tuning().prefill_last_only != 0;
+        AttnSegs d_sg_last = d_sg;
+        if (last_only) {
+            std::vector<int> q0_last(n_seqs), seg_last(n_seqs);
+            for (int i = 0; i < n_seqs; ++i) { seg_last[i] = i; q0_last[i] = (lens[i] - 1) / 64 * 64; }
+            d_sg_last.tile_seg = st.put(seg_last); d_sg_last.tile_q0 = st.put(q0_last);
+            if (!d_sg_last.tile_q0) return SA_ERR_NOMEM;
+        }
         if ((rc = st.flush(s))) return rc;
         hipLaunchKernelGGL(set_slot_state_kernel, dim3(cdiv(n_seqs, 256)), dim3(256), 0, s, d_slots, d_lens, kv_len, n_seqs);
-        if ((rc = decoder_layers_prefill(Ttot, d_tok_slot, d_tok_pos, &d_sg, (int)sg.tile_seg.size(), s))) return rc;
-        return heads(n_seqs, d_last, d_slots, 0, 0, false, s);
+        const T* head_src = dx;
+        if ((rc = decoder_layers_prefill(Ttot, d_tok_slot, d_tok_pos, &d_sg, (int)sg.tile_seg.size(), s, last_only ? &d_sg_last : nullptr,
+                                         n_seqs, d_last, n_seqs, &head_src))) return rc;
+        return heads(n_seqs, head_src, last_only ? nullptr : d_last, d_slots, 0, 0, false, s);
     }
 
     int set_active(const int32_t* slots, int n, hipStream_t s) override {
@@ -891,7 +938,7 @@
             if ((step == 0 || !fuse) && (rc = decode_embed(h))) return rc;
             for (int l = 0; l < c.dec_layers; ++l)
                 if ((rc = decode_layer(l, h))) return rc;
-            if ((rc = heads(M, nullptr, active_dev, step0 + step, 1, true, s, fuse && step + 1 < n_steps))) return rc;
+            if ((rc = heads(M, nullptr, nullptr, active_dev, step0 + step, 1, true, s, fuse && step + 1 < n_steps))) return rc;
         }
         return SA_OK;
     }
@@ -992,6 +1039,16 @@
         return SA_OK;
     }
 
+    int copy_kv_rows(int layer, int slot, int rows, void* k_out, void* v_out, hipStream_t s) override {
+        if (layer < 0 || layer >= c.dec_layers || slot < 0 || slot >= c.max_slots || rows <= 0 || rows > c.max_kv_len) return SA_ERR_ARG;
+        const int nkv = c.dec_kv_heads, d = c.dec_head_dim;
+        const size_t base = (((size_t)layer * c.max_slots + slot) * nkv) * c.max_kv_len * d;
+        const size_t pitch = (size_t)c.max_kv_len * d * sizeof(T), width = (size_t)rows * d * sizeof(T);
+        SA_HIP(hipMemcpy2DAsync(k_out, width, kcache + base, pitch, width, nkv, hipMemcpyDeviceToDevice, s));
+        SA_HIP(hipMemcpy2DAsync(v_out, width, vcache + base, pitch, width, nkv, hipMemcpyDeviceToDevice, s));
+        return SA_OK;
+    }
+
     int set_next_tokens(const int32_t* slots, const int32_t* toks, int n, hipStream_t s) override {
         if (n <= 0) return SA_OK;
         st_small.begin();
@@ -1131,6 +1188,10 @@
     if (!h || !dst || !rows || max_rows <= 0) return SA_ERR_ARG;
     return h->impl->copy_last_logits(dst, max_rows, rows, (hipStream_t)stream);
 }
+int surya_rec_copy_kv_rows(surya_rec* h, int layer, int slot, int rows, void* k_out, void* v_out, void* stream) {
+    if (!h || !k_out || !v_out) return SA_ERR_ARG;
+    return h->impl->copy_kv_rows(layer, slot, rows, k_out, v_out, (hipStream_t)stream);
+}
 int surya_rec_set_next_tokens(surya_rec* h, const int32_t* slots, const int32_t* tokens, int n, void* stream) {
     if (!h || !slots || !tokens) return SA_ERR_ARG;
     return h->impl->set_next_tokens(slots, tokens, n, (hipStream_t)stream);
@@ -1203,7 +1264,12 @@
                                         (bf16_t*)out, sg.a, q_row, q_head, k_row, k_head, o_row, o_head, group, causal, scale)
 #define SA_OPA_V(DD) hipLaunchKernelGGL((attn_valu_kernel<float, DD>), grid, dim3(256), 0, s, (const float*)q, (const float*)k, (const float*)v, \
                                         (float*)out, sg.a, q_row, q_head, k_row, k_head, o_row, o_head, group, causal, scale)
-    if (dtype == SA_DTYPE_BF16) {
+#define SA_OPA_O(DD, WW) hipLaunchKernelGGL((attn_mfma_occ_kernel<DD, WW>), grid, dim3(128), 0, s, (const bf16_t*)q, (const bf16_t*)k, (const bf16_t*)v, \
+                                            (bf16_t*)out, sg.a, q_row, q_head, k_row, k_head, o_row, o_head, group, causal, scale)
+    const int occ = tuning().enc_attn;
+    if (dtype == SA_DTYPE_BF16 && occ == 2 && (head_dim == 80 || head_dim == 128)) {
+        if (head_dim == 80) SA_OPA_O(80, 2); else SA_OPA_O(128, 2);
+    } else if (dtype == SA_DTYPE_BF16) {
         switch (head_dim) {
             case 32: SA_OPA_M(32); break;
             case 64: SA_OPA_M(64); break;
@@ -1224,6 +1290,7 @@
     }
 #undef SA_OPA_M
 #undef SA_OPA_V
+#undef SA_OPA_O
     SA_HIP(hipGetLastError());
     SA_HIP(hipStreamSynchronize(s));
     return SA_OK;
@@ -1395,7 +1462,8 @@
         {"graph", &t.graph}, {"split_target", &t.split_target}, {"split_min_kt", &t.split_min_kt}, {"split_max", &t.split_max},
         {"bigtile", &t.bigtile}, {"bigtile_any", &t.bigtile_any}, {"conv_lean", &t.conv_lean}, {"conv_persist", &t.conv_persist}, {"dwconv_pipe", &t.dwconv_pipe}, {"bigtile_ratio_pct", &t.bigtile_ratio_pct}, {"gateup_ring", &t.gateup_ring}, {"dring", &t.dring}, {"dring_min_kt", &t.dring_min_kt}, {"big_m_split", &t.big_m_split}, {"big_m_gateup", &t.big_m_gateup}, {"glds", &t.glds}, {"bigtile_min_k", &t.bigtile_min_k}, {"dattn", &t.dattn}, {"rnorm", &t.rnorm},
         {"ghead", &t.ghead}, {"fuse_embed", &t.fuse_embed}, {"persist", &t.persist}, {"lmhead", &t.lmhead}, {"kvprefetch", &t.kvprefetch},
-        {"dattn_db", &t.dattn_db}, {"lay_ln", &t.lay_ln}, {"det_head_blk", &t.det_head_blk}, {"det_fuse", &t.det_fuse}, {"det_up4", &t.det_up4}, {"fmb_chunk", &t.fmb_chunk}, {"ocrerr_cls_only", &t.ocrerr_cls_only}};
+        {"dattn_db", &t.dattn_db}, {"lay_ln", &t.lay_ln}, {"det_head_blk", &t.det_head_blk}, {"det_fuse", &t.det_fuse}, {"det_up4", &t.det_up4}, {"fmb_chunk", &t.fmb_chunk}, {"ocrerr_cls_only", &t.ocrerr_cls_only},
+        {"prefill_last_only", &t.prefill_last_only}, {"prefill_rope_epi", &t.prefill_rope_epi}, {"enc_attn", &t.enc_attn}};
     for (auto& e : tab)
         if (!strcmp(e.k, key)) {
             if (*e.v != value) ++tuning_epoch();
diff --git a/surya_amd/recognition/model.py b/surya_amd/recognition/model.py
--- a/surya_amd/recognition/model.py
+++ b/surya_amd/recognition/model.py
@@ -183,6 +183,14 @@
                                                self._stream), "surya_rec_encode_only")
         return out
 
+    def kv_rows(self, layer: int, slot: int, rows: int):
+        d = self.cfg.decoder
+        k = torch.empty((d.num_key_value_heads, rows, d.head_dim), dtype=self.dtype, device=self.device)
+        v = torch.empty_like(k)
+        L.check(self.lib.surya_rec_copy_kv_rows(self.handle, C.c_int(layer), C.c_int(slot), C.c_int(rows), L.ptr(k), L.ptr(v),
+                                                self._stream), "surya_rec_copy_kv_rows")
+        return k, v
+
     def last_logits(self) -> torch.Tensor:
         buf = torch.empty((self.max_slots, self.vocab), dtype=torch.float32, device=self.device)
         rows = C.c_int(0)
```
